# RainbowZL0/swin-unet-image-fusion

Measured on AMD Instinct MI355X. Metric: fused image-pairs/sec at 256x256, win=8, higher is better.
Workload: dtype bf16; 1 GPU; B=16/GPU 256x256 IR/visible pairs, win=8, 5-level Swin-UNet fusion forward (BASELINE configs[1]); global_batch=16, precision_mode=fast, residual_stream=fp32, hip_graph=True, steps_in_flight=3, kernel_schedule=throughput, collective=none, weights=random-init (numpy PCG64 recipe, seed 0)

## Files before the change

include/swinfuse.h:

```cpp
#ifndef SWINFUSE_H
#define SWINFUSE_H

#include <stddef.h>
#include <stdint.h>

#ifdef __cplusplus
extern "C" {
#endif

#define SWF_VERSION_MAJOR 0
#define SWF_VERSION_MINOR 1

typedef void* swf_stream_t;

typedef enum swf_status {
    SWF_OK = 0,
    SWF_ERR_NULL = -1,
    SWF_ERR_BAD_SHAPE = -2,
    SWF_ERR_PAD = -3,
    SWF_ERR_UNSUPPORTED = -4,
    SWF_ERR_WORKSPACE = -5,
    SWF_ERR_HIP = -6
} swf_status;

// ... 207 lines not shown
                const float* x_in, const float* y_in, float* x_out, float* y_out,
                int64_t tokens, int32_t channels, int32_t hidden,
                void* workspace, size_t workspace_bytes, swf_stream_t stream);

int swf_linear_fwd(const swf_linear* lin, const float* in, const float* residual, float* out,
                   int64_t tokens, int32_t n_in, int32_t n_out, int32_t act, swf_stream_t stream);
size_t swf_linear_workspace_bytes(int32_t precision, int64_t tokens, int32_t n_in, int32_t n_out);
int swf_linear_fwd_prec(const swf_linear* lin, int32_t precision, const float* in, const float* residual, float* out,
                        int64_t tokens, int32_t n_in, int32_t n_out, int32_t act,
                        void* workspace, size_t workspace_bytes, swf_stream_t stream);
int swf_layernorm_fwd(const swf_norm* ln, const float* in, float* out, int64_t tokens, int32_t C, int32_t elu,
                      swf_stream_t stream);
int swf_reflect_pad_fwd(const float* in, float* out, int32_t B, int32_t H, int32_t W, int32_t C,
                        int32_t pad_h, int32_t pad_w, swf_stream_t stream);
int swf_crop_fwd(const float* in, float* out, int32_t B, int32_t Hp, int32_t Wp, int32_t H, int32_t W, int32_t C,
                 swf_stream_t stream);

int swf_nchw_to_nhwc(const float* in, float* out, int32_t B, int32_t C, int32_t H, int32_t W, swf_stream_t stream);
int swf_nhwc_to_nchw(const float* in, float* out, int32_t B, int32_t C, int32_t H, int32_t W, swf_stream_t stream);

#define SWF_MAX_LEVELS 8
typedef struct swf_model_desc {
    int32_t levels;
    int32_t in_dims[SWF_MAX_LEVELS];
    int32_t out_dims[SWF_MAX_LEVELS];
    int32_t heads;
    int32_t head_dim[SWF_MAX_LEVELS];
    int32_t mlp_ratio;
    int32_t win_h, win_w, merge_h, merge_w;
    int32_t head_ksize;
    int32_t precision;
    int32_t schedule;
} swf_model_desc;

int32_t swf_model_param_count(const swf_model_desc* desc);
int swf_model_param_info(const swf_model_desc* desc, int32_t index, char* name_buf, size_t name_buf_len,
                         int64_t* offset_elems, int64_t* numel);
int64_t swf_model_arena_elems(const swf_model_desc* desc);
size_t swf_model_workspace_bytes(const swf_model_desc* desc, int32_t B, int32_t H, int32_t W);
int swf_model_forward(const swf_model_desc* desc, const float* arena, const float* ir, const float* vis,
                      float* out, int32_t B, int32_t H, int32_t W,
                      void* workspace, size_t workspace_bytes, swf_stream_t stream);

size_t swf_model_packed_bytes(const swf_model_desc* desc);
int swf_model_pack_weights(const swf_model_desc* desc, const float* arena, void* packed, size_t packed_bytes,
                           swf_stream_t stream);
int swf_model_forward_packed(const swf_model_desc* desc, const float* arena, const void* packed,
                             const float* ir, const float* vis, float* out, int32_t B, int32_t H, int32_t W,
                             void* workspace, size_t workspace_bytes, swf_stream_t stream);

int swf_model_forward_checked(const swf_model_desc* desc, const float* arena, const void* packed,
                              const float* ir, const float* vis, float* out, int32_t B, int32_t H, int32_t W,
                              void* workspace, size_t workspace_bytes, int32_t* cross_equal_flags, swf_stream_t stream);
int swf_model_forward_profiled(const swf_model_desc* desc, const float* arena, const void* packed,
                               const float* ir, const float* vis, float* out, int32_t B, int32_t H, int32_t W,
                               void* workspace, size_t workspace_bytes, float* seg_ms, int32_t seg_count, swf_stream_t stream);
int swf_tensors_equal(const float* a, const float* b, int64_t count, int32_t* flag, swf_stream_t stream);

int swf_bgr8_to_ycrcb_fwd(const uint8_t* bgr, float* y, float* crcb, int32_t B, int32_t H, int32_t W, swf_stream_t stream);
int swf_gray8_to_unit_fwd(const uint8_t* gray, float* out, int64_t count, swf_stream_t stream);
int swf_ycrcb_to_rgb_fwd(const float* fused_y, const float* crcb, float* rgb_f, uint8_t* rgb8,
                         int32_t B, int32_t H, int32_t W, swf_stream_t stream);

typedef struct swf_crop_row {
    uint64_t ir_off;
    uint64_t vis_off;
    int32_t H, W;
    int32_t top, left, h, w;
    int32_t flip;
    int32_t pad_;
} swf_crop_row;
size_t swf_paired_crop_rows_bytes(int32_t B);
int swf_paired_crop_rows_check(const swf_crop_row* rows_host, int32_t B, uint64_t ir_bytes, uint64_t vis_bytes);
int swf_paired_crop_resize_fwd(const uint8_t* ir_base, const uint8_t* vis_base, const swf_crop_row* rows_device, int32_t B,
                               int32_t out_h, int32_t out_w, float* ir_out, float* vis_y_out, swf_stream_t stream);

typedef struct swf_loss_desc {
    int32_t ssim_mode;
    int32_t use_psnr;
    float ir_ssim_weight, ir_psnr_weight;
    float ssim_scale, texture_scale, intensity_scale, psnr_scale;
    float ssim_ratio, texture_ratio, intensity_ratio, psnr_ratio;
} swf_loss_desc;
size_t swf_fusion_loss_workspace_bytes(const swf_loss_desc* desc, int32_t B, int32_t H, int32_t W, int32_t with_grad);
int swf_fusion_loss(const swf_loss_desc* desc, const float* fusion, const float* ir, const float* vis, float* terms, float* grad_fusion,
                    int32_t B, int32_t H, int32_t W, void* workspace, size_t workspace_bytes, swf_stream_t stream);

typedef struct swf_adam_desc {
    double beta1, beta2, eps, weight_decay;
    double max_grad_norm;
    int32_t norm_ready;
} swf_adam_desc;
typedef struct swf_adam_tensor {
    float* param; const float* grad; float* exp_avg; float* exp_avg_sq;
    int64_t numel;
    float step_size;
    float bc2_sqrt;
    int32_t first_chunk;
    int32_t reserved;
} swf_adam_tensor;
size_t swf_adam_table_bytes(int32_t n_tensors, int64_t total_elems);
int swf_adam_table_fill(void* table_host, size_t table_bytes, int32_t n_tensors, const void* const* param, const void* const* grad,
                        const void* const* exp_avg, const void* const* exp_avg_sq, const int64_t* numel, const float* step_size,
                        const float* bc2_sqrt);
int swf_adam_grad_norm(double max_grad_norm, const void* table_pinned_host, void* table_device, size_t table_bytes, int32_t n_tensors,
                       float* norm_out_device, swf_stream_t stream);
// ... 12 lines not shown
```

swin_unet_image_fusion_amd/_lib.py:

```python
from __future__ import annotations

import ctypes as C
import os
from typing import Optional

_HERE = os.path.dirname(os.path.abspath(__file__))
LIB_PATH = os.environ.get("SWF_LIB_PATH") or os.path.join(_HERE, "libswinfuse.so")

SWF_MAX_LEVELS = 8
PREC_FP32, PREC_FAST = 0, 1

OK, ERR_NULL, ERR_BAD_SHAPE, ERR_PAD, ERR_UNSUPPORTED, ERR_WORKSPACE, ERR_HIP = 0, -1, -2, -3, -4, -5, -6

c_float_p = C.c_void_p


class Linear(C.Structure):
    _fields_ = [("weight", C.c_void_p), ("bias", C.c_void_p)]


class Norm(C.Structure):
    _fields_ = [("gamma", C.c_void_p), ("beta", C.c_void_p)]


# ... 102 lines not shown
                                                _vp, _sz, _vp]),
    "swf_window_attention_bwd_drop": (C.c_int, [P(AttnDesc), P(AttnParams), _vp, _vp, _vp, _vp, _vp, _vp, _vp, P(AttnParams), _i32, _i32,
                                                _i32, P(Dropout), _i32, _vp, _sz, _vp]),
    "swf_mlp_drop_workspace_bytes": (_sz, [_i64, _i32, _i32]),
    "swf_mlp_fwd_drop": (C.c_int, [P(Linear), P(Linear), _vp, _vp, _i64, _i32, _i32, P(Dropout), _i32, _vp, _sz, _vp]),
    "swf_mlp_bwd_drop": (C.c_int, [P(Linear), P(Linear), _vp, _vp, _vp, P(Linear), P(Linear), _i64, _i32, _i32, P(Dropout), _i32,
                                   _vp, _sz, _vp]),
    "swf_layernorm_bwd_workspace_bytes": (_sz, [_i64, _i32]),
    "swf_layernorm_bwd": (C.c_int, [P(Norm), _vp, _vp, _vp, P(Norm), _i64, _i32, _vp, _sz, _vp]),
    "swf_patch_layer_bwd_workspace_bytes": (_sz, [_i32] * 8),
    "swf_patch_layer_bwd": (C.c_int, [P(PatchParams), _vp, _vp, _vp, P(PatchParams), _i32, _i32, _i32, _i32, _i32, _i32, _i32, _i32, _vp, _sz, _vp]),
    "swf_reflect_pad_bwd": (C.c_int, [_vp, _vp, _i32, _i32, _i32, _i32, _i32, _i32, _vp]),
    "swf_final_head_bwd_workspace_bytes": (_sz, [_i32, _i32, _i32, _i32]),
    "swf_final_head_bwd": (C.c_int, [P(HeadParams), _vp, _vp, _vp, _vp, _vp, P(HeadGrads), _i32, _i32, _i32, _i32, _i32, _vp, _sz, _vp]),
    "swf_final_head_batch_stats": (C.c_int, [P(HeadParams), _vp, _vp, _vp, _vp, _vp, _vp, C.c_float, _i32, _i32, _i32, _i32, _vp, _sz, _vp]),
    "swf_add_fwd": (C.c_int, [_vp, _vp, _vp, _i64, _vp]),
    "swf_block_pair4_fwd": (C.c_int, [P(BlockDesc), P(BlockStreamParams), P(BlockStreamParams), _vp, _vp, _vp, _vp, _i32, _i32, _i32, _vp, _sz, _vp]),
    "swf_patch_merge_fwd": (C.c_int, [P(PatchParams), _vp, _vp, _i32, _i32, _i32, _i32, _i32, _i32, _i32, _i32, _i32, _vp, _sz, _vp]),
    "swf_merge_out_shape": (C.c_int, [_i32, _i32, _i32, _i32, _i32, _i32, P(_i32), P(_i32), P(_i32), P(_i32)]),
    "swf_patch_unmerge_fwd": (C.c_int, [P(PatchParams), _vp, _vp, _vp, _i32, _i32, _i32, _i32, _i32, _i32, _i32, _i32, _i32, _i32, _i32, _vp, _sz, _vp]),
    "swf_patch_workspace_bytes": (_sz, [_i32] * 10),
    "swf_patch_merge_prec_workspace_bytes": (_sz, [_i32] * 11),
    "swf_patch_merge_fwd_prec": (C.c_int, [_i32, P(PatchParams), P(PatchParams), _vp, _vp, _vp, _vp] + [_i32] * 9
                                 + [P(PatchLn1), P(PatchLn1), P(_i32), _vp, _sz, _vp]),
    "swf_patch_unmerge_prec_workspace_bytes": (_sz, [_i32] * 13),
    "swf_patch_unmerge_fwd_prec": (C.c_int, [_i32, P(PatchParams), P(PatchParams), _vp, _vp, _vp, _vp, _vp, _vp] + [_i32] * 11
                                   + [P(PatchLn1), P(PatchLn1), P(_i32), _vp, _sz, _vp]),
    "swf_final_head_fwd": (C.c_int, [P(HeadParams), _vp, _vp, _vp, _i32, _i32, _i32, _i32, _vp, _sz, _vp]),
    "swf_linear_fwd": (C.c_int, [P(Linear), _vp, _vp, _vp, _i64, _i32, _i32, _i32, _vp]),
    "swf_mlp_workspace_bytes": (_sz, [_i32, _i64, _i32, _i32]),
    "swf_mlp_fwd": (C.c_int, [_i32, P(BlockStreamParams), P(BlockStreamParams), _vp, _vp, _vp, _vp, _i64, _i32, _i32, _vp, _sz, _vp]),
    "swf_linear_workspace_bytes": (_sz, [_i32, _i64, _i32, _i32]),
    "swf_linear_fwd_prec": (C.c_int, [P(Linear), _i32, _vp, _vp, _vp, _i64, _i32, _i32, _i32, _vp, _sz, _vp]),
    "swf_layernorm_fwd": (C.c_int, [P(Norm), _vp, _vp, _i64, _i32, _i32, _vp]),
    "swf_reflect_pad_fwd": (C.c_int, [_vp, _vp, _i32, _i32, _i32, _i32, _i32, _i32, _vp]),
    "swf_crop_fwd": (C.c_int, [_vp, _vp, _i32, _i32, _i32, _i32, _i32, _i32, _vp]),
    "swf_nchw_to_nhwc": (C.c_int, [_vp, _vp, _i32, _i32, _i32, _i32, _vp]),
    "swf_nhwc_to_nchw": (C.c_int, [_vp, _vp, _i32, _i32, _i32, _i32, _vp]),
    "swf_bgr8_to_ycrcb_fwd": (C.c_int, [_vp, _vp, _vp, _i32, _i32, _i32, _vp]),
    "swf_gray8_to_unit_fwd": (C.c_int, [_vp, _vp, _i64, _vp]),
    "swf_ycrcb_to_rgb_fwd": (C.c_int, [_vp, _vp, _vp, _vp, _i32, _i32, _i32, _vp]),
    "swf_paired_crop_rows_bytes": (_sz, [_i32]),
    "swf_paired_crop_rows_check": (C.c_int, [_vp, _i32, C.c_uint64, C.c_uint64]),
    "swf_paired_crop_resize_fwd": (C.c_int, [_vp, _vp, _vp, _i32, _i32, _i32, _vp, _vp, _vp]),
    "swf_model_param_count": (_i32, [P(ModelDesc)]),
    "swf_model_param_info": (C.c_int, [P(ModelDesc), _i32, C.c_char_p, _sz, P(_i64), P(_i64)]),
    "swf_model_arena_elems": (_i64, [P(ModelDesc)]),
    "swf_model_workspace_bytes": (_sz, [P(ModelDesc), _i32, _i32, _i32]),
    "swf_model_forward": (C.c_int, [P(ModelDesc), _vp, _vp, _vp, _vp, _i32, _i32, _i32, _vp, _sz, _vp]),
    "swf_model_packed_bytes": (_sz, [P(ModelDesc)]),
    "swf_model_pack_weights": (C.c_int, [P(ModelDesc), _vp, _vp, _sz, _vp]),
    "swf_model_forward_packed": (C.c_int, [P(ModelDesc), _vp, _vp, _vp, _vp, _vp, _i32, _i32, _i32, _vp, _sz, _vp]),
    "swf_model_forward_checked": (C.c_int, [P(ModelDesc), _vp, _vp, _vp, _vp, _vp, _i32, _i32, _i32, _vp, _sz, _vp, _vp]),
    "swf_model_forward_profiled": (C.c_int, [P(ModelDesc), _vp, _vp, _vp, _vp, _vp, _i32, _i32, _i32, _vp, _sz, P(C.c_float), _i32, _vp]),
    "swf_tensors_equal": (C.c_int, [_vp, _vp, _i64, _vp, _vp]),
    "swf_fusion_loss_workspace_bytes": (_sz, [P(LossDesc), _i32, _i32, _i32, _i32]),
    "swf_fusion_loss": (C.c_int, [P(LossDesc), _vp, _vp, _vp, _vp, _vp, _i32, _i32, _i32, _vp, _sz, _vp]),
    "swf_adam_table_bytes": (_sz, [_i32, _i64]),
    "swf_adam_table_fill": (C.c_int, [_vp, _sz, _i32, _vp, _vp, _vp, _vp, _vp, _vp, _vp]),
    "swf_adam_grad_norm": (C.c_int, [C.c_double, _vp, _vp, _sz, _i32, _vp, _vp]),
    "swf_adam_step": (C.c_int, [P(AdamDesc), _vp, _vp, _sz, _i32, _vp, _vp]),
}

_lib: Optional[C.CDLL] = None


class SwinFuseLibraryMissing(ImportError):
    pass


def lib() -> C.CDLL:
    global _lib
    if _lib is None:
        if not os.path.exists(LIB_PATH):
            raise SwinFuseLibraryMissing(
                f"{LIB_PATH} not found: build the HIP extension first "
                "(python -c 'import __graft_entry__ as g; g.build()').  There is no CPU fallback.")
        handle = C.CDLL(LIB_PATH)
        for name, (res, args) in SIGNATURES.items():
            fn = getattr(handle, name)
            fn.restype = res
            fn.argtypes = args
        _lib = handle
    return _lib


def check(status: int) -> None:
    if status == OK:
        return
    msg = lib().swf_last_error_string().decode(errors="replace")
    kind = lib().swf_status_string(status).decode()
    text = f"libswinfuse: {kind}: {msg}"
    if status == ERR_BAD_SHAPE:
        raise ValueError(text)
    if status == ERR_UNSUPPORTED:
        raise NotImplementedError(text)
    raise RuntimeError(text)
```

swin_unet_image_fusion_amd/csrc/kernels_patchrr.h:

```cpp
#pragma once
#include "kernels_patch.h"

namespace swf {

bool patch_rr_supported(int decoder, int Cin, int Cout, int mh, int mw);
size_t patch_rr_packed_bytes(int decoder, int Cin, int Cout, int mh, int mw);
int pack_patch_rr(int decoder, int Cin, int Cout, int mh, int mw, const float* weight, const float* bias, const float* gamma,
                  const float* beta, void* dst, hipStream_t stream);
int launch_patch_rr(const PatchFusedDesc& d, const void* const* packed, int nstream, hipStream_t stream);

}
```

swin_unet_image_fusion_amd/csrc/kernels_patchrr.hip:

```cpp
#include "kernels_patchrr.h"

#include <algorithm>

#include "win_frag.h"

namespace swf {
namespace {

using namespace wf;

struct PrrArgs {
    const float* in[2]; float* out[2]; const float* skip[2]; const char* packed[2];
    int B, H, W, Cin;
    int mh, mw, Hm, Wm;
    int Ho, Wo;
    int K, N, Cout, M;
};

template <int KS, int NT>
struct PRR {
    static constexpr int NFRAG = NT * KS * 2;
    static constexpr int NV = NT * 16;
    static constexpr size_t p_vec = size_t(NFRAG) * 1024;
    static constexpr size_t p_total = p_vec + size_t(3) * 2 * NV * 4;
// ... 158 lines not shown
            for (int nt = 0; nt < NT; ++nt)
#pragma unroll
                for (int i = 0; i < 16; ++i) {
                    const float d = acc[u][nt][i] - mean;
                    q += (32 * nt + rho(i, hf) < N) ? d * d : 0.f;
                }
            const float rstd = __builtin_amdgcn_rsqf(sum_halves(q) * invN + 1e-5f);
            const int t = tok[u];
            if constexpr (DEC_VEC) {
                if (a.Cout > 1) {
                    if constexpr (!SKIP_EARLY) load_skips(u);
                }
            }
#pragma unroll
            for (int nt = 0; nt < NT; ++nt)
#pragma unroll
                for (int g = 0; g < 4; ++g) {
                    const int n0 = 32 * nt + 8 * g + 4 * hf;
                    if (n0 < N) {
                        float y[4];
#pragma unroll
                        for (int j = 0; j < 4; ++j) {
                            const int i = 4 * g + j;
                            const float z = (acc[u][nt][i] - mean) * rstd * vgam[nt * 16 + i] + vbet[nt * 16 + i];
                            y[j] = z > 0.f ? z : __builtin_amdgcn_exp2f(z * kLog2e) - 1.0f;
                        }
                        if constexpr (!DEC) {
                            if (live[u]) *reinterpret_cast<float4*>(a.out[s] + (int64_t)t * N + n0) = make_float4(y[0], y[1], y[2], y[3]);
                        } else if (a.Cout == 1) {
                            if (live[u]) {
                                const int mx = t % a.Wm, t2 = t / a.Wm, my = t2 % a.Hm, b = t2 / a.Hm;
#pragma unroll
                                for (int j = 0; j < 4; ++j) {
                                    const int yy = my * 2 + (j >> 1), xx = mx * 2 + (j & 1);
                                    if (yy < a.Ho && xx < a.Wo) {
                                        const int64_t o = ((int64_t)b * a.Ho + yy) * a.Wo + xx;
                                        a.out[s][o] = a.skip[s] ? y[j] + a.skip[s][o] : y[j];
                                    }
                                }
                            }
                        } else {
                            const int o = oidx[u][nt][g];
                            if (o >= 0) {
                                const float4 k4 = skv[u][nt][g];
                                *reinterpret_cast<float4*>(a.out[s] + o) = make_float4(y[0] + k4.x, y[1] + k4.y, y[2] + k4.z, y[3] + k4.w);
                            }
                        }
                    }
                }
        }
    }
}

struct PrrPackArgs { const float* w; const float* bias; const float* gamma; const float* beta; char* dst; int K, N; };

template <int KS, int NT>
__global__ __launch_bounds__(256) void patch_rr_pack_kernel(PrrPackArgs a) {
    using P = PRR<KS, NT>;
    const int gtid = blockIdx.x * blockDim.x + threadIdx.x, gsz = gridDim.x * blockDim.x;
    for (int idx = gtid; idx < P::NFRAG * 512; idx += gsz) {
        const int f = idx >> 9, lane = (idx >> 3) & 63, e = idx & 7, r = lane & 31, hf = lane >> 5;
        const int hl = f & 1, ks = (f >> 1) % KS, nt = f / (2 * KS);
        const int n = 32 * nt + r, k = 16 * ks + 8 * hf + e;
        const float val = (n < a.N && k < a.K) ? a.w[(int64_t)n * a.K + k] : 0.f;
        const bf16 hi = (bf16)val;
        reinterpret_cast<bf16*>(a.dst)[idx] = hl ? (bf16)(val - (float)hi) : hi;
    }
    float* vec = reinterpret_cast<float*>(a.dst + P::p_vec);
    for (int i = gtid; i < 3 * 2 * P::NV; i += gsz) {
        const int which = i / (2 * P::NV), hf = (i / P::NV) & 1, j = i % P::NV, nt = j >> 4, reg = j & 15;
        const int n = 32 * nt + rho(reg, hf);
        const float* src = which == 0 ? a.bias : which == 1 ? a.gamma : a.beta;
        vec[i] = (n < a.N && src) ? src[n] : 0.f;
    }
}

bool shape_class(int decoder, int Cin, int Cout, int mh, int mw, int* ks, int* nt) {
    if (mh != 2 || mw != 2 || Cin <= 0 || Cout <= 0) return false;
    const int K = decoder ? Cin : 4 * Cin, N = decoder ? 4 * Cout : Cout;
    if (decoder) {
        if (Cin % 8 || !(Cout == 1 || Cout % 4 == 0)) return false;
    } else {
        if (!(Cin == 1 || Cin % 8 == 0) || Cout % 4) return false;
    }
    *ks = (K + 15) / 16;
    *nt = (N + 31) / 32;
    const int k = *ks, n = *nt;
    if (decoder) return (k == 2 && n == 1) || (k == 3 && n == 3) || (k == 6 && n == 6);
    return (k == 1 && n == 1 && Cin == 1) || (k == 6 && n == 2) || (k == 12 && n == 3);
}

template <int KS, int NT, int DEC, int CIN1, int TPW>
int launch_t(const PrrArgs& a, int nstream, hipStream_t stream) {
    const int ngroup = (a.M + 32 * TPW - 1) / (32 * TPW);
    const int gx = std::max(1, std::min((ngroup + 3) / 4, 8 * num_cus() / nstream));
    hipLaunchKernelGGL((patch_rr_kernel<KS, NT, DEC, CIN1, TPW>), dim3(gx, nstream), dim3(256), 0, stream, a);
    return check_launch("patch_rr");
}

}

bool patch_rr_supported(int decoder, int Cin, int Cout, int mh, int mw) {
    int ks, nt;
    return shape_class(decoder, Cin, Cout, mh, mw, &ks, &nt);
}

size_t patch_rr_packed_bytes(int decoder, int Cin, int Cout, int mh, int mw) {
    int ks, nt;
    if (!shape_class(decoder, Cin, Cout, mh, mw, &ks, &nt)) return 0;
    return align_up(size_t(nt) * ks * 2 * 1024 + size_t(3) * 2 * nt * 16 * 4, 256);
}

int pack_patch_rr(int decoder, int Cin, int Cout, int mh, int mw, const float* weight, const float* bias, const float* gamma,
                  const float* beta, void* dst, hipStream_t stream) {
    int ks, nt;
    if (!shape_class(decoder, Cin, Cout, mh, mw, &ks, &nt)) return fail(SWF_ERR_UNSUPPORTED, "pack_patch_rr: shape not covered");
    PrrPackArgs a{weight, bias, gamma, beta, static_cast<char*>(dst), decoder ? Cin : 4 * Cin, decoder ? 4 * Cout : Cout};
#define SWF_PRR_PACK(KS_, NT_) if (ks == KS_ && nt == NT_) { hipLaunchKernelGGL((patch_rr_pack_kernel<KS_, NT_>), dim3(32), dim3(256), 0, stream, a); return check_launch("pack_patch_rr"); }
    SWF_PRR_PACK(1, 1) SWF_PRR_PACK(2, 1) SWF_PRR_PACK(3, 3) SWF_PRR_PACK(6, 2) SWF_PRR_PACK(6, 6) SWF_PRR_PACK(12, 3)
#undef SWF_PRR_PACK
    return fail(SWF_ERR_UNSUPPORTED, "pack_patch_rr: shape class");
}

int launch_patch_rr(const PatchFusedDesc& d, const void* const* packed, int nstream, hipStream_t stream) {
    int ks, nt;
    if (!shape_class(d.decoder, d.Cin, d.Cout, d.mh, d.mw, &ks, &nt)) return fail(SWF_ERR_UNSUPPORTED, "patch_rr: shape not covered");
    if (d.M <= 0 || d.M > INT32_MAX - 64) return fail(SWF_ERR_UNSUPPORTED, "patch_rr: token count");
    const int64_t in_elems = (int64_t)d.B * d.H * d.W * d.Cin;
    const int64_t out_elems = d.decoder ? (int64_t)d.B * d.Ho * d.Wo * d.Cout : d.M * (int64_t)d.N;
    if (in_elems >= (int64_t(1) << 31) || out_elems >= (int64_t(1) << 31)) return fail(SWF_ERR_UNSUPPORTED, "patch_rr: tensor too large");
    PrrArgs a{};
    uintptr_t bits = 0;
    for (int s = 0; s < nstream; ++s) {
        if (!packed || !packed[s]) return fail(SWF_ERR_NULL, "patch_rr: packed image missing");
        a.in[s] = d.in[s]; a.out[s] = d.out[s]; a.skip[s] = d.skip[s]; a.packed[s] = static_cast<const char*>(packed[s]);
        bits |= reinterpret_cast<uintptr_t>(d.in[s]) | reinterpret_cast<uintptr_t>(d.out[s]) | reinterpret_cast<uintptr_t>(d.skip[s]) |
                reinterpret_cast<uintptr_t>(packed[s]);
    }
    if (bits % 16) return fail(SWF_ERR_UNSUPPORTED, "patch_rr: tensors must be 16-byte aligned");
    a.B = d.B; a.H = d.H; a.W = d.W; a.Cin = d.Cin; a.mh = d.mh; a.mw = d.mw; a.Hm = d.Hm; a.Wm = d.Wm; a.Ho = d.Ho; a.Wo = d.Wo;
    a.K = d.K; a.N = d.N; a.Cout = d.Cout; a.M = (int)d.M;
    if (!d.decoder) {
        if (ks == 1 && nt == 1 && d.Cin == 1) return launch_t<1, 1, 0, 1, 2>(a, nstream, stream);
        if (ks == 6 && nt == 2) return launch_t<6, 2, 0, 0, 2>(a, nstream, stream);
        if (ks == 12 && nt == 3) return launch_t<12, 3, 0, 0, 1>(a, nstream, stream);
    } else {
        if (ks == 2 && nt == 1) return launch_t<2, 1, 1, 0, 2>(a, nstream, stream);
        if (ks == 3 && nt == 3) return launch_t<3, 3, 1, 0, 1>(a, nstream, stream);
        if (ks == 6 && nt == 6) return launch_t<6, 6, 1, 0, 1>(a, nstream, stream);
    }
    return fail(SWF_ERR_UNSUPPORTED, "patch_rr: no instantiation for k-steps %d, tiles %d (decoder %d)", ks, nt, d.decoder);
}

}
```

swin_unet_image_fusion_amd/csrc/kernels_win24.hip:

```cpp
#include "win_host.h"

namespace swf {
namespace {

using namespace wf;

constexpr int W24_WAVES = 3;

template <int HID_>
struct G24 {
    static constexpr int C = 24, HID = HID_, HEADS = 8, D = 3;
    static constexpr bool ONES_H = HID % 32 != 0;
    static constexpr int NT1 = (HID + (ONES_H ? 1 : 0) + 31) / 32;
    static constexpr int KU = (HID + (ONES_H ? 1 : 0) + 15) / 16;
    static constexpr int F_QKV = 0;
    static constexpr int F_P = 12;
    static constexpr int F_W1 = 16;
    static constexpr int F_W2 = F_W1 + 4 * NT1;
    static constexpr int NFRAG = F_W2 + 2 * KU;
    static constexpr size_t p_vec = size_t(NFRAG) * 1024;
    static constexpr int V_LN1G = 0, V_LN1B = 12, V_LN2G = 24, V_LN2B = 36, V_B2 = 48;
    static constexpr size_t p_bias = p_vec + 2 * 64 * 4;
    static constexpr size_t p_total = p_bias + size_t(2) * 2 * 16 * 64 * 4;
    static constexpr size_t l_k = 0, l_v = l_k + 16 * 1024, l_vec = l_v + 16 * 1024, l_total = l_vec + 2 * 2 * 64 * 4;
    static constexpr size_t p_total16 = p_bias + size_t(15) * 64 * 16 * 4;
    static constexpr size_t l_k16 = 0, l_v16 = 32 * 1024, l_vec16 = 64 * 1024, l_total16 = l_vec16 + 2 * 2 * 64 * 4;
};

__device__ __forceinline__ void layernorm_frags(const f32x16& res, const float* vec, int goff, int boff, u32x4 (&xh)[2], u32x4 (&xl)[2]) {
    float s = 0.f;
#pragma unroll
    for (int i = 0; i < 12; ++i) s += res[i];
    const float mean = sum_halves(s) * (1.0f / 24.0f);
    float d[12], q = 0.f;
#pragma unroll
    for (int i = 0; i < 12; ++i) {
        d[i] = res[i] - mean;
        q += d[i] * d[i];
    }
    const float rstd = __builtin_amdgcn_rsqf(sum_halves(q) * (1.0f / 24.0f) + 1e-5f);
    float n[16];
#pragma unroll
    for (int a = 0; a < 3; ++a) {
        const float4 g = *reinterpret_cast<const float4*>(vec + goff + 4 * a);
        const float4 b = *reinterpret_cast<const float4*>(vec + boff + 4 * a);
        n[4 * a + 0] = d[4 * a + 0] * rstd * g.x + b.x;
        n[4 * a + 1] = d[4 * a + 1] * rstd * g.y + b.y;
        n[4 * a + 2] = d[4 * a + 2] * rstd * g.z + b.z;
        n[4 * a + 3] = d[4 * a + 3] * rstd * g.w + b.w;
    }
    n[12] = 1.0f;
    n[13] = n[14] = n[15] = 0.f;
    split8(n, xh[0], xl[0]);
    split8(n + 8, xh[1], xl[1]);
}

__device__ __forceinline__ void raw_frags(const f32x16& res, u32x4 (&xh)[2], u32x4 (&xl)[2]) {
    float n[16];
#pragma unroll
    for (int i = 0; i < 12; ++i) n[i] = res[i];
// ... 43 lines not shown
            float p[8];
#pragma unroll
            for (int j = 0; j < 8; ++j) p[j] = __builtin_amdgcn_exp2f((ps >> 1) ? s1[8 * (ps & 1) + j] : s0[8 * (ps & 1) + j]);
            const u32x4 pf = pack8_f16(p);
            const u32x4 va = vsrc[ps * 64];
            t = mfma_f16(va, pf, ps == 0 ? zero16 : t);
            __builtin_amdgcn_sched_barrier(0);
        }
#pragma unroll
        for (int j = 0; j < 4; ++j) {
            const int i = 4 * (h >> 1) + j;
            o[i] = keep ? (ONLINE ? __builtin_fmaf(o[i], alpha, t[i]) : t[i]) : o[i];
        }
        __builtin_amdgcn_sched_barrier(0);
    }
    return o;
}

__device__ __forceinline__ void load_rows24(const __amdgpu_buffer_rsrc_t& irs, unsigned tokoff, f32x16& dstv) {
#pragma unroll
    for (int a = 0; a < 3; ++a) {
        const f32x4 v = __builtin_bit_cast(f32x4, __builtin_amdgcn_raw_buffer_load_b128(irs, tokoff, 32 * a, 0));
        dstv[4 * a] = v.x; dstv[4 * a + 1] = v.y; dstv[4 * a + 2] = v.z; dstv[4 * a + 3] = v.w;
    }
    dstv[12] = dstv[13] = dstv[14] = dstv[15] = 0.f;
}
__device__ __forceinline__ void store_rows24(__amdgpu_buffer_rsrc_t ors, unsigned tokoff, f32x16 res) {
#pragma unroll
    for (int a = 0; a < 3; ++a) {
        const f32x4 v = {res[4 * a], res[4 * a + 1], res[4 * a + 2], res[4 * a + 3]};
        __builtin_amdgcn_raw_buffer_store_b128(__builtin_bit_cast(u32x4, v), ors, tokoff, 32 * a, 0);
    }
}

template <class G, class WFn>
__device__ __forceinline__ f32x16 project24(WFn WF, f32x16 o, f32x16 res) {
    float t[16];
#pragma unroll
    for (int a = 0; a < 4; ++a) {
        const float inv = __builtin_amdgcn_rcpf(o[4 * a + 3]);
        t[4 * a] = o[4 * a] * inv; t[4 * a + 1] = o[4 * a + 1] * inv; t[4 * a + 2] = o[4 * a + 2] * inv;
        t[4 * a + 3] = 1.0f;
    }
    u32x4 oh[2], ol[2];
    split8(t, oh[0], ol[0]);
    split8(t + 8, oh[1], ol[1]);
    SWF_WF_FENCE();
#pragma unroll
    for (int s = 0; s < 2; ++s) res = mma3(WF(G::F_P + 2 * s), WF(G::F_P + 2 * s + 1), oh[s], ol[s], res);
    return res;
}


template <int HID, int WS, int MODE = WIN_BLOCK, bool RAW = false>
__global__ __launch_bounds__(256, W24_WAVES) void window24_kernel(WinArgs args) {
    using G = G24<HID>;
    static_assert(WS == 7 || WS == 8, "window side");
    static_assert(MODE == WIN_BLOCK || MODE == WIN_ATTN || MODE == WIN_MLP, "mode");
    static_assert(!RAW || MODE != WIN_BLOCK, "RAW belongs to the half-block modes");
    constexpr bool ATT = MODE != WIN_MLP, MLP = MODE != WIN_ATTN;
    __shared__ __attribute__((aligned(16))) char smem[G::l_total];
    u32x4* kimg = reinterpret_cast<u32x4*>(smem + G::l_k);
    u32x4* vimg = reinterpret_cast<u32x4*>(smem + G::l_v);
    float* lvec = reinterpret_cast<float*>(smem + G::l_vec);

    const int tid = threadIdx.x, lane = tid & 63, wave = tid >> 6;
    const int ws = wave >> 1, qb = wave & 1, r = lane & 31, hf = lane >> 5;
    const int H = args.H, W = args.W, nwx = MLP && !ATT ? 1 : W / WS, nwy = MLP && !ATT ? 1 : H / WS, npi = nwx * nwy;
    const int nwin = ATT ? args.B * npi : (max(args.ntok[0], args.ntok[1]) + 63) / 64;
    const int sh = args.shift ? WS / 2 : 0;
    const int kvs = args.cross ? 1 - ws : ws;

    for (int i = tid; i < 2 * 2 * 64; i += 256) lvec[i] = reinterpret_cast<const float*>(args.packed[i >> 7] + G::p_vec)[i & 127];
    const __amdgpu_buffer_rsrc_t wrs = __builtin_amdgcn_make_buffer_rsrc(const_cast<char*>(uniform_ptr(args.packed[ws])), 0, (int)G::p_total, 0x00020000);
    const __amdgpu_buffer_rsrc_t krs = __builtin_amdgcn_make_buffer_rsrc(const_cast<char*>(uniform_ptr(args.packed[kvs])), 0, (int)G::p_total, 0x00020000);
    const int act_bytes = ATT ? args.B * H * W * 24 * 4 : args.ntok[ws] * 24 * 4;
    const __amdgpu_buffer_rsrc_t irs = __builtin_amdgcn_make_buffer_rsrc(const_cast<float*>(uniform_ptr(args.in[ws])), 0, act_bytes, 0x00020000);
    const __amdgpu_buffer_rsrc_t ors = __builtin_amdgcn_make_buffer_rsrc(uniform_ptr(args.out[ws]), 0, (MODE == WIN_BLOCK || args.out[ws]) ? act_bytes : 0, 0x00020000);
    const unsigned loff = (unsigned)lane * 16u;
    auto WF = [&](int f) { return __builtin_bit_cast(u32x4, __builtin_amdgcn_raw_buffer_load_b128(wrs, loff, f * 1024, 0)); };
    auto WK = [&](int f) { return __builtin_bit_cast(u32x4, __builtin_amdgcn_raw_buffer_load_b128(krs, loff, f * 1024, 0)); };
    const float* vec = lvec + (ws * 2 + hf) * 64;
    f32x16 bias[2];
    auto load_bias = [&]() {
        const int vo = lane * 128 + qb * (2 * 16 * 64 * 4);
#pragma unroll
        for (int kt = 0; kt < 2; ++kt)
#pragma unroll
            for (int q4 = 0; q4 < 4; ++q4) {
                const f32x4 t = __builtin_bit_cast(f32x4, __builtin_amdgcn_raw_buffer_load_b128(wrs, vo + (kt * 16 + q4 * 4) * 4, (int)G::p_bias, 0));
#pragma unroll
                for (int e = 0; e < 4; ++e) bias[kt][q4 * 4 + e] = t[e];
            }
    };
    if constexpr (ATT) load_bias();
    const bool half1 = hf != 0;
    const bool col_masked = half1 != (((r >> 2) & 1) != 0);
    __syncthreads();

    int it = 0;
    for (int win = blockIdx.x; win < nwin; win += gridDim.x, ++it) {
        SWF_WF_FENCE();
        const int b = win / npi, wrem = win - b * npi;
        const int wy = wrem / nwx, wx = wrem - wy * nwx;
        const int buf = it & 1;
        int lane_w = lane;
        asm volatile("" : "+v"(lane_w));
        const int ty = 4 * qb + ((lane_w >> 3) & 3), tx = lane_w & 7;
        unsigned oy = wy * WS + ty + sh, ox = wx * WS + tx + sh;
        oy = oy < oy - (unsigned)H ? oy : oy - (unsigned)H;
        ox = ox < ox - (unsigned)W ? ox : ox - (unsigned)W;
        const unsigned tokoff = [&]() -> unsigned {
            if constexpr (ATT) {
                return (WS == 8 || (ty < WS && tx < WS)) ? (unsigned)((((b * H + (int)oy) * W + (int)ox) * 24 + 4 * (lane_w >> 5)) * 4) : 0x80000000u;
            } else {
                const int tok = 64 * win + 32 * qb + (lane_w & 31);
                return tok < args.ntok[ws] ? (unsigned)((tok * 24 + 4 * (lane_w >> 5)) * 4) : 0x80000000u;
            }
        }();
        const f32x16 zero16 = {0.f, 0.f, 0.f, 0.f, 0.f, 0.f, 0.f, 0.f, 0.f, 0.f, 0.f, 0.f, 0.f, 0.f, 0.f, 0.f};

        f32x16 res;
        if constexpr (ATT) {
        u32x4 qf[2];
        {
            f32x16 x0;
            load_rows24(irs, tokoff, x0);
            u32x4 xh[2], xl[2];
            if constexpr (RAW) raw_frags(x0, xh, xl);
            else layernorm_frags(x0, vec, G::V_LN1G, G::V_LN1B, xh, xl);
            f32x16 acc = zero16;
            if (!(RAW && ws == 1)) {
#pragma unroll
                for (int s = 0; s < 2; ++s) acc = mma3(WF(G::F_QKV + 2 * s), WF(G::F_QKV + 2 * s + 1), xh[s], xl[s], acc);
                float t[16];
#pragma unroll
                for (int i = 0; i < 16; ++i) t[i] = acc[i];
                qf[0] = pack8_f16(t);
                qf[1] = pack8_f16(t + 8);
            }
            SWF_WF_FENCE();
            if (!(RAW && ws == 0)) {
                float t[16];
                acc = zero16;
#pragma unroll
                for (int s = 0; s < 2; ++s) acc = mma3(WK(G::F_QKV + 4 + 2 * s), WK(G::F_QKV + 5 + 2 * s), xh[s], xl[s], acc);
#pragma unroll
                for (int i = 0; i < 16; ++i) t[i] = acc[i];
                u32x4* kdst = kimg + (((buf * 2 + kvs) * 2 + qb) * 2) * 64 + lane;
                kdst[0] = pack8_f16(t);
// ... 19 lines not shown
            const u32x4* vsrc = vimg + ((buf * 2 + ws) * 4) * 64 + lane;
            if (rowv || colv) {
                const float pen0 = ((rowv && qb == 1) || (colv && col_masked)) ? -INFINITY : 0.f;
                const float pen1 = ((rowv && qb == 0) || (colv && col_masked)) ? -INFINITY : 0.f;
#pragma unroll
                for (int i = 0; i < 16; ++i) { bias[0][i] += pen0; bias[1][i] += pen1; }
            }
            o = attention24<false>(ksrc, vsrc, qf, bias, half1, zero16);
            if (rowv || colv) load_bias();
        }

        SWF_WF_FENCE();
        if constexpr (RAW) res = zero16;
        else load_rows24(irs, tokoff, res);
        res = project24<G>(WF, o, res);
        } else {
            load_rows24(irs, tokoff, res);
        }

        if constexpr (MLP) {
            u32x4 xh[2], xl[2];
            if constexpr (RAW) { raw_frags(res, xh, xl); res = zero16; }
            else layernorm_frags(res, vec, G::V_LN2G, G::V_LN2B, xh, xl);
#pragma unroll
            for (int tI = 0; tI < G::NT1; ++tI) {
                SWF_WF_FENCE();
                f32x16 acc = zero16;
#pragma unroll
                for (int s = 0; s < 2; ++s)
                    acc = mma3(WF(G::F_W1 + 4 * tI + 2 * s), WF(G::F_W1 + 4 * tI + 2 * s + 1), xh[s], xl[s], acc);
                float e[16];
                elu_tile(acc, e);
#pragma unroll
                for (int s2 = 0; s2 < 2; ++s2) {
                    const int u = 2 * tI + s2;
                    if (u < G::KU) {
                        u32x4 hh, hl;
                        split8(e + 8 * s2, hh, hl);
                        SWF_WF_FENCE();
                        res = mma3(WF(G::F_W2 + 2 * u), WF(G::F_W2 + 2 * u + 1), hh, hl, res);
                    }
                }
                __builtin_amdgcn_sched_barrier(0);
            }
            if constexpr (!G::ONES_H) {
#pragma unroll
                for (int a = 0; a < 3; ++a) {
                    const float4 b2 = *reinterpret_cast<const float4*>(vec + G::V_B2 + 4 * a);
                    res[4 * a] += b2.x; res[4 * a + 1] += b2.y; res[4 * a + 2] += b2.z; res[4 * a + 3] += b2.w;
                }
            }
        }

        store_rows24(ors, tokoff, res);
    }

    if (args.warm[0]) warm_next_block<256>(args, tid);
}

template <int HID>
__global__ __launch_bounds__(256, 2) void window24w16_kernel(WinArgs args) {
    using G = G24<HID>;
    extern __shared__ __attribute__((aligned(16))) char smem16[];
    u32x4* kimg = reinterpret_cast<u32x4*>(smem16 + G::l_k16);
    u32x4* vimg = reinterpret_cast<u32x4*>(smem16 + G::l_v16);
    float* lvec = reinterpret_cast<float*>(smem16 + G::l_vec16);

    const int tid = threadIdx.x, lane = tid & 63, wave = tid >> 6;
    const int ws = wave >> 1, pw = wave & 1, r = lane & 31, hf = lane >> 5;
    const int H = args.H, W = args.W, nwx = W / 16, nwy = H / 16, npi = nwx * nwy;
    const int nwin = args.B * npi;
    const int sh = args.shift ? 8 : 0;
    const int kvs = args.cross ? 1 - ws : ws;

    for (int i = tid; i < 2 * 2 * 64; i += 256) lvec[i] = reinterpret_cast<const float*>(args.packed[i >> 7] + G::p_vec)[i & 127];
    const __amdgpu_buffer_rsrc_t wrs = __builtin_amdgcn_make_buffer_rsrc(const_cast<char*>(uniform_ptr(args.packed[ws])), 0, (int)G::p_total16, 0x00020000);
    const __amdgpu_buffer_rsrc_t krs = __builtin_amdgcn_make_buffer_rsrc(const_cast<char*>(uniform_ptr(args.packed[kvs])), 0, (int)G::p_total16, 0x00020000);
    const int act_bytes = args.B * H * W * 24 * 4;
    const __amdgpu_buffer_rsrc_t irs = __builtin_amdgcn_make_buffer_rsrc(const_cast<float*>(uniform_ptr(args.in[ws])), 0, act_bytes, 0x00020000);
    const __amdgpu_buffer_rsrc_t ors = __builtin_amdgcn_make_buffer_rsrc(uniform_ptr(args.out[ws]), 0, act_bytes, 0x00020000);
    const unsigned loff = (unsigned)lane * 16u;
    auto WF = [&](int f) { return __builtin_bit_cast(u32x4, __builtin_amdgcn_raw_buffer_load_b128(wrs, loff, f * 1024, 0)); };
    auto WK = [&](int f) { return __builtin_bit_cast(u32x4, __builtin_amdgcn_raw_buffer_load_b128(krs, loff, f * 1024, 0)); };
    const float* vec = lvec + (ws * 2 + hf) * 64;
    const bool half1 = hf != 0;
    const f32x16 zero16 = {0.f, 0.f, 0.f, 0.f, 0.f, 0.f, 0.f, 0.f, 0.f, 0.f, 0.f, 0.f, 0.f, 0.f, 0.f, 0.f};
    __syncthreads();

    for (int win = blockIdx.x; win < nwin; win += gridDim.x) {
        SWF_WF_FENCE();
        const int b = win / npi, wrem = win - b * npi;
        const int wy = wrem / nwx, wx = wrem - wy * nwx;
        auto tokoff_of = [&](int j) {
            int lane_w = lane;
            asm volatile("" : "+v"(lane_w));
            unsigned oy = wy * 16 + 2 * j + ((lane_w >> 4) & 1) + sh, ox = wx * 16 + (lane_w & 15) + sh;
            oy = oy < oy - (unsigned)H ? oy : oy - (unsigned)H;
            ox = ox < ox - (unsigned)W ? ox : ox - (unsigned)W;
            return (unsigned)((((b * H + (int)oy) * W + (int)ox) * 24 + 4 * (lane_w >> 5)) * 4);
        };

        u32x4 qf[4][2];
#pragma unroll
        for (int q = 0; q < 4; ++q) { qf[q][0] = u32x4{0u, 0u, 0u, 0u}; qf[q][1] = u32x4{0u, 0u, 0u, 0u}; }
        {
            u32x4 wq[4], wk[4], wv[4];
#pragma unroll
// ... 123 lines not shown
        if (f < G::F_P) {
            const int t = f >> 2, st = (f >> 1) & 1;
            hl = f & 1;
            const int k = rho(8 * st + e, hf), head = r >> 2, c = r & 3;
            const swf_linear& l = t == 0 ? p.attn.q : t == 1 ? p.attn.k : p.attn.v;
            if (c < 3) {
                const int row = 3 * head + c;
                val = k < 24 ? lin(l, row, k, 24) : (k == 24 ? pack_bia(l, row) : 0.f);
                if (t == 0) val *= qscale;
            } else if (t != 0 && k == 24) {
                val = 1.0f;
            }
        } else if (f < G::F_W1) {
            const int st = ((f - G::F_P) >> 1) & 1;
            hl = f & 1;
            const int k = rho(8 * st + e, hf), head = k >> 2, c = k & 3;
            if (r < 24) val = c < 3 ? lin(p.attn.proj, r, 3 * head + c, 24) : (k == 3 ? pack_bia(p.attn.proj, r) : 0.f);
        } else if (f < G::F_W2) {
            const int g = f - G::F_W1, t = g >> 2, st = (g >> 1) & 1;
            hl = g & 1;
            const int k = rho(8 * st + e, hf), hid = 32 * t + r;
            if (hid < HID) val = (k < 24 ? lin(p.fc1, hid, k, 24) : (k == 24 ? pack_bia(p.fc1, hid) : 0.f)) * kLog2e;
            else if (G::ONES_H && hid == HID && k == 24) val = 1.0f;
        } else {
            const int g = f - G::F_W2, u = g >> 1;
            hl = g & 1;
            const int hid = 32 * (u >> 1) + rho(8 * (u & 1) + e, hf);
            if (r < 24) val = hid < HID ? lin(p.fc2, r, hid, HID) * kLn2 : ((G::ONES_H && hid == HID) ? pack_bia(p.fc2, r) : 0.f);
        }
        const bf16 hi = (bf16)val;
        reinterpret_cast<bf16*>(dst)[idx] = hl ? (bf16)(val - (float)hi) : hi;
    }
    float* vec = reinterpret_cast<float*>(dst + G::p_vec);
    for (int i = gtid; i < 128; i += gsz) {
        const int hf = i >> 6, j = i & 63, which = j / 12, k = j % 12;
        const int c = 8 * (k >> 2) + 4 * hf + (k & 3);
        float v = 0.f;
        if (which == 0) v = p.ln1.gamma ? p.ln1.gamma[c] : 1.f;
        else if (which == 1) v = p.ln1.beta ? p.ln1.beta[c] : 0.f;
        else if (which == 2) v = p.ln2.gamma ? p.ln2.gamma[c] : 1.f;
        else if (which == 3) v = p.ln2.beta ? p.ln2.beta[c] : 0.f;
        else if (which == 4) v = (p.fc2.weight && p.fc2.bias) ? p.fc2.bias[c] : 0.f;
        vec[i] = v;
    }
    if (p.attn.bias_table) pack_rel_bias<true>(reinterpret_cast<float*>(dst + G::p_bias), p.attn.bias_table, a.ws, gtid, gsz);
}

struct L24 {
    static constexpr int C = 24, D = 3, HID_WIDE = 96, HID_NARROW = 4, PACK_GRID = 32, WAVES = W24_WAVES;
    static constexpr const char *name = "win24", *pack_name = "pack_win24";
    template <int HID> using G = G24<HID>;
    template <int HID>
    static void pack(dim3 grid, const WinPackArgs& a, hipStream_t stream) { hipLaunchKernelGGL((pack24_kernel<HID>), grid, dim3(256), 0, stream, a); }
    template <int HID, int WS, int MODE, bool RAW>
    static int launch(const swf_block_desc&, const WinArgs& a, int grid, hipStream_t stream) {
        hipLaunchKernelGGL((window24_kernel<HID, WS, MODE, RAW>), dim3(grid), dim3(256), 0, stream, a);
        return check_launch(MODE == WIN_BLOCK ? "window24" : "window24 (half block)");
    }
    template <int HID>
    static int launch16(const WinArgs& a, int nwin, hipStream_t stream) {
        constexpr int lds = (int)G24<HID>::l_total16;
        SWF_TRY(raise_lds_limit<&window24w16_kernel<HID>>(lds, "window24w16"));
        hipLaunchKernelGGL((window24w16_kernel<HID>), dim3(std::min(nwin, 2 * num_cus())), dim3(256), lds, stream, a);
        return check_launch("window24w16");
    }
};

}

const WinLevel& win24_level() {
    static const WinLevel level = win_level<L24>();
    return level;
}

}
```

swin_unet_image_fusion_amd/csrc/kernels_win48.hip:

```cpp
#include "win_host.h"

namespace swf {
namespace {

using namespace wf;

constexpr int W48_WAVES = 2;

template <int HID_>
struct G48 {
    static constexpr int C = 48, HID = HID_, HEADS = 8, D = 6;
    static constexpr int NT1 = HID / 32, KU = HID / 16;
    static_assert(HID % 32 == 0, "hidden tiles");
    static constexpr int F_QKV = 0;
    static constexpr int F_P = 36;
    static constexpr int F_W1 = 52;
    static constexpr int F_W2 = F_W1 + 6 * NT1;
    static constexpr int NFRAG = F_W2 + 4 * KU;
    static constexpr int V_LN1G = 0, V_LN1B = 24, V_LN2G = 48, V_LN2B = 72, V_B2 = 96, V_BQ = 120, V_BK = 152, V_B1 = 184, VHF = 288;
    static_assert(V_B1 + 16 * NT1 <= VHF, "vector block");
    static constexpr int VSTREAM = 2 * VHF + 64;
    static constexpr size_t p_vec = size_t(NFRAG) * 1024;
    static constexpr size_t p_bias = (p_vec + size_t(VSTREAM) * 4 + 15) / 16 * 16;
    static constexpr size_t p_total = p_bias + size_t(2) * 2 * 16 * 64 * 4;
    static constexpr size_t l_k = 0, l_v = 16 * 1024, l_vec = 32 * 1024, l_total = l_vec + size_t(2) * VSTREAM * 4;
    static constexpr size_t p_total16 = p_bias + size_t(15) * 16 * 64 * 4;
    static constexpr size_t l_k16 = 0, l_v16 = 32 * 1024, l_vec16 = 64 * 1024, l_total16 = l_vec16 + size_t(2) * VSTREAM * 4;
};


__device__ __forceinline__ void raw48(const f32x16& x0, const f32x16& x1, u32x4 (&xh)[3], u32x4 (&xl)[3]) {
    float n[24];
#pragma unroll
    for (int i = 0; i < 24; ++i) n[i] = i < 16 ? x0[i] : x1[i - 16];
    split8(n, xh[0], xl[0]);
    split8(n + 8, xh[1], xl[1]);
    split8(n + 16, xh[2], xl[2]);
}

__device__ __forceinline__ void layernorm48(const f32x16& x0, const f32x16& x1, const float* vec, int goff, int boff, u32x4 (&xh)[3], u32x4 (&xl)[3]) {
    float s = 0.f;
#pragma unroll
    for (int i = 0; i < 16; ++i) s += x0[i];
#pragma unroll
    for (int i = 0; i < 8; ++i) s += x1[i];
    const float mean = sum_halves(s) * (1.0f / 48.0f);
    float d[24], q = 0.f;
#pragma unroll
    for (int i = 0; i < 24; ++i) {
        d[i] = (i < 16 ? x0[i] : x1[i - 16]) - mean;
        q += d[i] * d[i];
    }
    const float rstd = __builtin_amdgcn_rsqf(sum_halves(q) * (1.0f / 48.0f) + 1e-5f);
    float n[24];
#pragma unroll
    for (int a = 0; a < 6; ++a) {
        const float4 g = *reinterpret_cast<const float4*>(vec + goff + 4 * a);
        const float4 b = *reinterpret_cast<const float4*>(vec + boff + 4 * a);
        n[4 * a + 0] = d[4 * a + 0] * rstd * g.x + b.x;
        n[4 * a + 1] = d[4 * a + 1] * rstd * g.y + b.y;
// ... 12 lines not shown
    if constexpr (!ONLINE) { o[0] = zero16; o[1] = zero16; }
#pragma unroll
    for (int h = 0; h < 8; ++h) {
        const int T = h >> 2, hq = h & 3, sp = hq >> 1, sub = hq & 1;
        const u32x4 ka0 = ksrc[((0 * 2 + T) * 2 + sp) * 64], ka1 = ksrc[((1 * 2 + T) * 2 + sp) * 64];
        u32x4 qm = {0u, 0u, 0u, 0u};
        qm[2 * sub] = qf[T][sp][2 * sub];
        qm[2 * sub + 1] = qf[T][sp][2 * sub + 1];
        float mx;
        {
            f32x16 s0 = mfma_f16(ka0, qm, bias[0]);
            mx = max3f(s0[0], s0[1], s0[2]);
#pragma unroll
            for (int i = 3; i < 15; i += 2) mx = max3f(mx, s0[i], s0[i + 1]);
            mx = __builtin_fmaxf(mx, s0[15]);
        }
        {
            f32x16 s1 = mfma_f16(ka1, qm, bias[1]);
#pragma unroll
            for (int i = 0; i < 16; i += 2) mx = max3f(mx, s1[i], s1[i + 1]);
        }
        mx = max_halves(mx);
        f16 nm = (f16)(-mx);
        float alpha = 0.f;
        if constexpr (ONLINE) {
            const float mold = mrun[h];
            nm = (f16)(-__builtin_fmaxf(mold, mx));
            const float mnew = -(float)nm;
            alpha = __builtin_amdgcn_exp2f(mold - mnew);
            mrun[h] = mnew;
        }
        qm[2 * sub + 1] |= half1 ? ((unsigned)__builtin_bit_cast(unsigned short, nm) << 16) : 0u;
        f32x16 t;
#pragma unroll
        for (int kt = 0; kt < 2; ++kt) {
            f32x16 sc = mfma_f16(kt ? ka1 : ka0, qm, bias[kt]);
#pragma unroll
            for (int s2 = 0; s2 < 2; ++s2) {
                float p[8];
#pragma unroll
                for (int j = 0; j < 8; ++j) p[j] = __builtin_amdgcn_exp2f(sc[8 * s2 + j]);
                const u32x4 pf = pack8_f16(p);
                const u32x4 va = vsrc[(T * VSTEPS + 2 * kt + s2) * 64];
                t = mfma_f16(va, pf, (kt == 0 && s2 == 0) ? zero16 : t);
                __builtin_amdgcn_sched_barrier(0);
            }
        }
#pragma unroll
        for (int j = 0; j < 4; ++j) o[T][4 * hq + j] = ONLINE ? __builtin_fmaf(o[T][4 * hq + j], alpha, t[4 * hq + j]) : t[4 * hq + j];
        __builtin_amdgcn_sched_barrier(0);
    }
}

template <int HID, int WS, int MODE = WIN_BLOCK, bool RAW = false>
__global__ __launch_bounds__(256, W48_WAVES) void window48_kernel(WinArgs args) {
    using G = G48<HID>;
    static_assert(WS == 7 || WS == 8, "window side");
    static_assert(!RAW || MODE != WIN_BLOCK, "RAW belongs to the half-block modes");
    constexpr bool ATT = MODE != WIN_MLP, MLP = MODE != WIN_ATTN;
    __shared__ __attribute__((aligned(16))) char smem[G::l_total];
    u32x4* kimg = reinterpret_cast<u32x4*>(smem + G::l_k);
    u32x4* vimg = reinterpret_cast<u32x4*>(smem + G::l_v);
    float* lvec = reinterpret_cast<float*>(smem + G::l_vec);

    const int tid = threadIdx.x, lane = tid & 63, wave = tid >> 6;
    const int ws = wave >> 1, qb = wave & 1, r = lane & 31, hf = lane >> 5;
    const int H = args.H, W = args.W, nwx = ATT ? W / WS : 1, nwy = ATT ? H / WS : 1, npi = nwx * nwy;
    const int nwin = ATT ? args.B * npi : (max(args.ntok[0], args.ntok[1]) + 63) / 64;
    const int sh = args.shift ? WS / 2 : 0;
    const int kvs = args.cross ? 1 - ws : ws;

    const __amdgpu_buffer_rsrc_t wrs = __builtin_amdgcn_make_buffer_rsrc(const_cast<char*>(uniform_ptr(args.packed[ws])), 0, (int)G::p_total, 0x00020000);
    const __amdgpu_buffer_rsrc_t krs = __builtin_amdgcn_make_buffer_rsrc(const_cast<char*>(uniform_ptr(args.packed[kvs])), 0, (int)G::p_total, 0x00020000);
    const int act_bytes = ATT ? args.B * H * W * 48 * 4 : args.ntok[ws] * 48 * 4;
    const __amdgpu_buffer_rsrc_t irs = __builtin_amdgcn_make_buffer_rsrc(const_cast<float*>(uniform_ptr(args.in[ws])), 0, act_bytes, 0x00020000);
    const __amdgpu_buffer_rsrc_t ors = __builtin_amdgcn_make_buffer_rsrc(uniform_ptr(args.out[ws]), 0, (MODE == WIN_BLOCK || args.out[ws]) ? act_bytes : 0, 0x00020000);
    const unsigned loff = (unsigned)lane * 16u;
    auto WF = [&](int f) { return __builtin_bit_cast(u32x4, __builtin_amdgcn_raw_buffer_load_b128(wrs, loff, f * 1024, 0)); };
    auto WK = [&](int f) { return __builtin_bit_cast(u32x4, __builtin_amdgcn_raw_buffer_load_b128(krs, loff, f * 1024, 0)); };
    const float* vec = lvec + ws * G::VSTREAM + hf * G::VHF;
    const float* veck = lvec + kvs * G::VSTREAM + hf * G::VHF;
    const float* vecv = lvec + kvs * G::VSTREAM + 2 * G::VHF;
    const bool half1 = hf != 0;
    const bool col_masked = half1 != (((r >> 2) & 1) != 0);
    const f32x16 zero16 = {0.f, 0.f, 0.f, 0.f, 0.f, 0.f, 0.f, 0.f, 0.f, 0.f, 0.f, 0.f, 0.f, 0.f, 0.f, 0.f};

    for (int win = blockIdx.x; win < nwin; win += gridDim.x) {
        SWF_WF_FENCE();
        const int b = win / npi, wrem = win - b * npi;
        const int wy = wrem / nwx, wx = wrem - wy * nwx;
        const int ty = 4 * qb + (r >> 3), tx = r & 7;
        int oy = wy * WS + ty + sh, ox = wx * WS + tx + sh;
        oy = oy >= H ? oy - H : oy;
        ox = ox >= W ? ox - W : ox;
        const unsigned tokoff = [&]() -> unsigned {
            if constexpr (ATT) {
                return (WS == 8 || (ty < WS && tx < WS)) ? (unsigned)((((b * H + oy) * W + ox) * 48 + 4 * hf) * 4) : 0x80000000u;
            } else {
                const int tok = 64 * win + 32 * qb + r;
                return tok < args.ntok[ws] ? (unsigned)((tok * 48 + 4 * hf) * 4) : 0x80000000u;
            }
        }();
        auto load_rows = [&](f32x16& t0, f32x16& t1) {
#pragma unroll
            for (int a = 0; a < 6; ++a) {
                const f32x4 v = __builtin_bit_cast(f32x4, __builtin_amdgcn_raw_buffer_load_b128(irs, tokoff, 32 * a, 0));
                if (a < 4) { t0[4 * a] = v.x; t0[4 * a + 1] = v.y; t0[4 * a + 2] = v.z; t0[4 * a + 3] = v.w; }
                else { t1[4 * (a - 4)] = v.x; t1[4 * (a - 4) + 1] = v.y; t1[4 * (a - 4) + 2] = v.z; t1[4 * (a - 4) + 3] = v.w; }
            }
#pragma unroll
            for (int i = 8; i < 16; ++i) t1[i] = 0.f;
        };

        f32x16 res0, res1;
        if constexpr (ATT) {
        u32x4 qf[2][2];
        {
            u32x4 wq[2][6];
            auto req = [&](int ph, u32x4 (&dst)[6]) {
                const int m = ph >> 1, T = ph & 1;
#pragma unroll
                for (int i = 0; i < 6; ++i) dst[i] = m == 0 ? WF(G::F_QKV + ((m * 2 + T) * 3) * 2 + i) : WK(G::F_QKV + ((m * 2 + T) * 3) * 2 + i);
            };
            req(0, wq[0]);
            f32x16 x0, x1;
            load_rows(x0, x1);
            if (win == (int)blockIdx.x) {
                static_assert(G::VSTREAM % 4 == 0 && G::p_vec % 16 == 0, "vector sections move as 16-byte groups");
                    fill_vectors<G::VSTREAM / 4, 256>(lvec, args.packed[0] + G::p_vec, args.packed[1] + G::p_vec, tid);
                __syncthreads();
            }
            u32x4 xh[3], xl[3];
            if constexpr (RAW) raw48(x0, x1, xh, xl);
            else layernorm48(x0, x1, vec, G::V_LN1G, G::V_LN1B, xh, xl);
            float t[16];
#pragma unroll
            for (int ph = 0; ph < 6; ++ph) {
                const int m = ph >> 1, T = ph & 1;
                SWF_WF_FENCE();
                if (ph + 1 < 6) req(ph + 1, wq[(ph + 1) & 1]);
                SWF_WF_FENCE();
                const u32x4 (&w)[6] = wq[ph & 1];
                f32x16 acc = zero16;
                if (RAW && (m == 0 ? ws == 1 : ws == 0)) {
                    if (ph == 2 && win != (int)blockIdx.x) __syncthreads();
                } else if (m < 2) {
#pragma unroll
                    for (int s = 0; s < 3; ++s) acc = mma3(w[2 * s], w[2 * s + 1], xh[s], xl[s], acc);
                    const float* bsrc = m == 0 ? vec + G::V_BQ : veck + G::V_BK;
#pragma unroll
                    for (int g = 0; g < 4; ++g) {
                        const float4 bb = *reinterpret_cast<const float4*>(bsrc + 16 * T + 4 * g);
                        t[4 * g] = acc[4 * g] + bb.x; t[4 * g + 1] = acc[4 * g + 1] + bb.y; t[4 * g + 2] = acc[4 * g + 2] + bb.z; t[4 * g + 3] = acc[4 * g + 3] + bb.w;
                    }
                    if (m == 0) {
                        qf[T][0] = pack8_f16(t);
                        qf[T][1] = pack8_f16(t + 8);
                    } else {
                        if (T == 0 && win != (int)blockIdx.x) __syncthreads();
                        u32x4* kdst = kimg + (((kvs * 2 + qb) * 2 + T) * 2) * 64 + lane;
                        kdst[0] = pack8_f16(t);
                        kdst[64] = pack8_f16(t + 8);
                    }
                } else {
#pragma unroll
                    for (int s = 0; s < 3; ++s) acc = mma3(xh[s], xl[s], w[2 * s], w[2 * s + 1], acc);
                    const float bv = vecv[32 * T + r];
#pragma unroll
                    for (int i = 0; i < 16; ++i) t[i] = acc[i] + bv;
                    u32x4* vdst = vimg + ((kvs * 2 + T) * 4 + 2 * qb) * 64 + lane;
                    vdst[0] = pack8_f16(t);
                    vdst[64] = pack8_f16(t + 8);
                }
            }
        }
        f32x16 bias[2];
        load_bias_tiles(wrs, loff, (int)G::p_bias, __builtin_amdgcn_readfirstlane(qb) * 2, bias);
        __syncthreads();
        if (RAW && ws == 1) continue;

        f32x16 o[2];
        {
            const bool rowv = args.shift && wy == nwy - 1, colv = args.shift && wx == nwx - 1;
            const u32x4* ksrc = kimg + (ws * 8) * 64 + lane;
            const u32x4* vsrc = vimg + (ws * 8) * 64 + lane;
            if (rowv || colv) {
                const float pen0 = ((rowv && qb == 1) || (colv && col_masked)) ? -INFINITY : 0.f;
                const float pen1 = ((rowv && qb == 0) || (colv && col_masked)) ? -INFINITY : 0.f;
#pragma unroll
                for (int i = 0; i < 16; ++i) { bias[0][i] += pen0; bias[1][i] += pen1; }
            }
            attention48<false>(ksrc, vsrc, qf, bias, half1, o);
        }

        u32x4 wpj[16];
        SWF_WF_FENCE();
        if constexpr (RAW) { res0 = zero16; res1 = zero16; }
        else load_rows(res0, res1);
#pragma unroll
        for (int i = 0; i < 16; ++i) wpj[i] = WF(G::F_P + i);
        SWF_WF_FENCE();
        {
            u32x4 oh[4], ol[4];
#pragma unroll
            for (int T = 0; T < 2; ++T) {
                float t[16];
#pragma unroll
                for (int q = 0; q < 4; ++q) {
                    float lo_, den;
                    halves(o[T][4 * q + 2], lo_, den);
                    const float inv = __builtin_amdgcn_rcpf(den);
                    t[4 * q] = o[T][4 * q] * inv; t[4 * q + 1] = o[T][4 * q + 1] * inv; t[4 * q + 2] = o[T][4 * q + 2] * inv; t[4 * q + 3] = o[T][4 * q + 3] * inv;
                }
                split8(t, oh[2 * T], ol[2 * T]);
                split8(t + 8, oh[2 * T + 1], ol[2 * T + 1]);
            }
#pragma unroll
            for (int ks = 0; ks < 4; ++ks) {
                res0 = mma3(wpj[(0 * 4 + ks) * 2], wpj[(0 * 4 + ks) * 2 + 1], oh[ks], ol[ks], res0);
                res1 = mma3(wpj[(1 * 4 + ks) * 2], wpj[(1 * 4 + ks) * 2 + 1], oh[ks], ol[ks], res1);
            }
        }

        } else {
            load_rows(res0, res1);
            if (win == (int)blockIdx.x) {
                fill_vectors<G::VSTREAM / 4, 256>(lvec, args.packed[0] + G::p_vec, args.packed[1] + G::p_vec, tid);
                __syncthreads();
            }
        }

        if constexpr (MLP) {
            u32x4 w1[2][6];
            auto req1 = [&](int tI, u32x4 (&dst)[6]) {
#pragma unroll
                for (int i = 0; i < 6; ++i) dst[i] = WF(G::F_W1 + tI * 6 + i);
            };
            u32x4 w2[2][2][2][2];
            auto req2 = [&](int tI, u32x4 (&dst)[2][2][2]) {
#pragma unroll
                for (int To = 0; To < 2; ++To)
#pragma unroll
                    for (int s2 = 0; s2 < 2; ++s2) {
                        dst[To][s2][0] = WF(G::F_W2 + (To * G::KU + 2 * tI + s2) * 2);
                        dst[To][s2][1] = WF(G::F_W2 + (To * G::KU + 2 * tI + s2) * 2 + 1);
                    }
            };
            req1(0, w1[0]);
            req2(0, w2[0]);
            u32x4 xh[3], xl[3];
            if constexpr (RAW) { raw48(res0, res1, xh, xl); res0 = zero16; res1 = zero16; }
            else layernorm48(res0, res1, vec, G::V_LN2G, G::V_LN2B, xh, xl);
#pragma unroll
            for (int tI = 0; tI < G::NT1; ++tI) {
                SWF_WF_FENCE();
                if (tI + 1 < G::NT1) { req1(tI + 1, w1[(tI + 1) & 1]); req2(tI + 1, w2[(tI + 1) & 1]); }
                SWF_WF_FENCE();
                const u32x4 (&w)[6] = w1[tI & 1];
                f32x16 acc = zero16;
#pragma unroll
                for (int s = 0; s < 3; ++s) acc = mma3(w[2 * s], w[2 * s + 1], xh[s], xl[s], acc);
                float e[16];
                elu_tile(acc, vec + G::V_B1 + 16 * tI, e);
#pragma unroll
                for (int s2 = 0; s2 < 2; ++s2) {
                    u32x4 hh, hl;
                    split8(e + 8 * s2, hh, hl);
                    res0 = mma3(w2[tI & 1][0][s2][0], w2[tI & 1][0][s2][1], hh, hl, res0);
                    res1 = mma3(w2[tI & 1][1][s2][0], w2[tI & 1][1][s2][1], hh, hl, res1);
                }
                __builtin_amdgcn_sched_barrier(0);
            }
#pragma unroll
            for (int a = 0; a < 6; ++a) {
                const float4 b2 = *reinterpret_cast<const float4*>(vec + G::V_B2 + 4 * a);
                if (a < 4) { res0[4 * a] += b2.x; res0[4 * a + 1] += b2.y; res0[4 * a + 2] += b2.z; res0[4 * a + 3] += b2.w; }
                else { res1[4 * (a - 4)] += b2.x; res1[4 * (a - 4) + 1] += b2.y; res1[4 * (a - 4) + 2] += b2.z; res1[4 * (a - 4) + 3] += b2.w; }
            }
        }

#pragma unroll
        for (int a = 0; a < 6; ++a) {
            const f32x4 v = a < 4 ? f32x4{res0[4 * a], res0[4 * a + 1], res0[4 * a + 2], res0[4 * a + 3]}
                                  : f32x4{res1[4 * (a - 4)], res1[4 * (a - 4) + 1], res1[4 * (a - 4) + 2], res1[4 * (a - 4) + 3]};
            __builtin_amdgcn_raw_buffer_store_b128(__builtin_bit_cast(u32x4, v), ors, tokoff, 32 * a, 0);
        }
    }

    if (args.warm[0]) warm_next_block<256>(args, tid);
}

template <int HID>
__global__ __launch_bounds__(256, 2) void window48w16_kernel(WinArgs args) {
    using G = G48<HID>;
    extern __shared__ __attribute__((aligned(16))) char smem48[];
    u32x4* kimg = reinterpret_cast<u32x4*>(smem48 + G::l_k16);
    u32x4* vimg = reinterpret_cast<u32x4*>(smem48 + G::l_v16);
    float* lvec = reinterpret_cast<float*>(smem48 + G::l_vec16);

    const int tid = threadIdx.x, lane = tid & 63, wave = tid >> 6;
    const int ws = blockIdx.y, r = lane & 31, hf = lane >> 5;
    const int H = args.H, W = args.W, nwx = W / 16, nwy = H / 16, npi = nwx * nwy;
    const int nwin = args.B * npi;
    const int sh = args.shift ? 8 : 0;
    const int src = args.cross ? 1 - ws : ws;

    static_assert(G::VSTREAM % 4 == 0 && G::p_vec % 16 == 0, "vector sections move as 16-byte groups");
                    fill_vectors<G::VSTREAM / 4, 256>(lvec, args.packed[0] + G::p_vec, args.packed[1] + G::p_vec, tid);
    const __amdgpu_buffer_rsrc_t wrs = __builtin_amdgcn_make_buffer_rsrc(const_cast<char*>(args.packed[ws]), 0, (int)G::p_total16, 0x00020000);
    const int act_bytes = args.B * H * W * 48 * 4;
    const __amdgpu_buffer_rsrc_t irs = __builtin_amdgcn_make_buffer_rsrc(const_cast<float*>(args.in[ws]), 0, act_bytes, 0x00020000);
    const __amdgpu_buffer_rsrc_t srs = __builtin_amdgcn_make_buffer_rsrc(const_cast<float*>(args.in[src]), 0, act_bytes, 0x00020000);
    const __amdgpu_buffer_rsrc_t ors = __builtin_amdgcn_make_buffer_rsrc(args.out[ws], 0, act_bytes, 0x00020000);
    const unsigned loff = (unsigned)lane * 16u;
    auto WF = [&](int f) { return __builtin_bit_cast(u32x4, __builtin_amdgcn_raw_buffer_load_b128(wrs, loff, f * 1024, 0)); };
    const float* vec = lvec + ws * G::VSTREAM + hf * G::VHF;
    const float* vecs = lvec + src * G::VSTREAM + hf * G::VHF;
    const float* vecv = lvec + ws * G::VSTREAM + 2 * G::VHF;
    const bool half1 = hf != 0;
    const f32x16 zero16 = {0.f, 0.f, 0.f, 0.f, 0.f, 0.f, 0.f, 0.f, 0.f, 0.f, 0.f, 0.f, 0.f, 0.f, 0.f, 0.f};
    __syncthreads();

    for (int win = blockIdx.x; win < nwin; win += gridDim.x) {
        SWF_WF_FENCE();
        const int b = win / npi, wrem = win - b * npi;
        const int wy = wrem / nwx, wx = wrem - wy * nwx;
        auto tokoff_of = [&](int j) {
            int oy = wy * 16 + 2 * j + (r >> 4) + sh, ox = wx * 16 + (r & 15) + sh;
            oy = oy >= H ? oy - H : oy;
            ox = ox >= W ? ox - W : ox;
            return (unsigned)((((b * H + oy) * W + ox) * 48 + 4 * hf) * 4);
        };
        auto load_rows = [&](const __amdgpu_buffer_rsrc_t& rs, unsigned tokoff, f32x16& t0, f32x16& t1) {
#pragma unroll
            for (int a = 0; a < 6; ++a) {
                const f32x4 v = __builtin_bit_cast(f32x4, __builtin_amdgcn_raw_buffer_load_b128(rs, tokoff, 32 * a, 0));
                if (a < 4) { t0[4 * a] = v.x; t0[4 * a + 1] = v.y; t0[4 * a + 2] = v.z; t0[4 * a + 3] = v.w; }
                else { t1[4 * (a - 4)] = v.x; t1[4 * (a - 4) + 1] = v.y; t1[4 * (a - 4) + 2] = v.z; t1[4 * (a - 4) + 3] = v.w; }
// ... 198 lines not shown
        } else if (f < G::F_W1) {
            const int g = (f - G::F_P) >> 1, ks = g & 3, To = g >> 2;
            hl = f & 1;
            const int n = 32 * To + r, v = kslot(ks, hf, e), head = v >> 3, c = v & 7;
            if (n < 48) val = c < 6 ? pack_wgt(p.attn.proj, n * 48 + head * 6 + c) : (v == 6 ? pack_bia(p.attn.proj, n) : 0.f);
        } else if (f < G::F_W2) {
            const int g = (f - G::F_W1) >> 1, s = g % 3, tI = g / 3;
            hl = f & 1;
            const int k = kslot(s, hf, e), hid = 32 * tI + r;
            if (k < 48) val = pack_wgt(p.fc1, hid * 48 + k) * kLog2e;
        } else {
            const int g = (f - G::F_W2) >> 1, u = g % G::KU, To = g / G::KU;
            hl = f & 1;
            const int n = 32 * To + r, hid = kslot(u, hf, e);
            if (n < 48) val = pack_wgt(p.fc2, n * HID + hid) * kLn2;
        }
        const bf16 hi = (bf16)val;
        reinterpret_cast<bf16*>(dst)[idx] = hl ? (bf16)(val - (float)hi) : hi;
    }
    float* vec = reinterpret_cast<float*>(dst + G::p_vec);
    for (int i = gtid; i < G::VSTREAM; i += gsz) {
        float v = 0.f;
        if (i < 2 * G::VHF) {
            const int hf = i / G::VHF, j = i % G::VHF;
            if (j < G::V_BQ) {
                const int which = j / 24, k = j % 24;
                const int c = k < 16 ? rho(k, hf) : 32 + rho(k - 16, hf);
                v = which == 0 ? (p.ln1.gamma ? p.ln1.gamma[c] : 1.f) : which == 1 ? (p.ln1.beta ? p.ln1.beta[c] : 0.f)
                  : which == 2 ? (p.ln2.gamma ? p.ln2.gamma[c] : 1.f) : which == 3 ? (p.ln2.beta ? p.ln2.beta[c] : 0.f) : pack_bia(p.fc2, c);
            } else if (j < G::V_B1) {
                const int isk = j >= G::V_BK, k = (j - (isk ? G::V_BK : G::V_BQ)), T = k >> 4, vch = 32 * T + rho(k & 15, hf);
                const int head = vch >> 3, c = vch & 7;
                if (c < 6) v = isk ? pack_bia(p.attn.k, head * 6 + c) : pack_bia(p.attn.q, head * 6 + c) * qscale;
                else if (isk && c == 7) v = 1.0f;
            } else if (j < G::V_B1 + 16 * G::NT1) {
                const int k = j - G::V_B1, hid = 32 * (k >> 4) + rho(k & 15, hf);
                v = pack_bia(p.fc1, hid) * kLog2e;
            }
        } else {
            const int vch = i - 2 * G::VHF, head = vch >> 3, c = vch & 7;
            v = c < 6 ? pack_bia(p.attn.v, head * 6 + c) : (c == 6 ? 1.0f : 0.f);
        }
        vec[i] = v;
    }
    if (p.attn.bias_table) pack_rel_bias<false>(reinterpret_cast<float*>(dst + G::p_bias), p.attn.bias_table, a.ws, gtid, gsz);
}

struct L48 {
    static constexpr int C = 48, D = 6, HID_WIDE = 192, HID_NARROW = 96, PACK_GRID = 64, WAVES = W48_WAVES;
    static constexpr const char *name = "win48", *pack_name = "pack_win48";
    template <int HID> using G = G48<HID>;
    template <int HID>
    static void pack(dim3 grid, const WinPackArgs& a, hipStream_t stream) { hipLaunchKernelGGL((pack48_kernel<HID>), grid, dim3(256), 0, stream, a); }
    template <int HID, int WS, int MODE, bool RAW>
    static int launch(const swf_block_desc&, const WinArgs& a, int grid, hipStream_t stream) {
        hipLaunchKernelGGL((window48_kernel<HID, WS, MODE, RAW>), dim3(grid), dim3(256), 0, stream, a);
        return check_launch(MODE == WIN_BLOCK ? "window48" : "window48 (half block)");
    }
    template <int HID>
    static int launch16(const WinArgs& a, int nwin, hipStream_t stream) {
        constexpr int lds = (int)G48<HID>::l_total16;
        SWF_TRY(raise_lds_limit<&window48w16_kernel<HID>>(lds, "window48w16"));
        hipLaunchKernelGGL((window48w16_kernel<HID>), dim3(std::min(nwin, num_cus()), 2), dim3(256), lds, stream, a);
        return check_launch("window48w16");
    }
};

}

const WinLevel& win48_level() {
    static const WinLevel level = win_level<L48>();
    return level;
}

}
```

swin_unet_image_fusion_amd/csrc/kernels_win96.hip:

```cpp
#include "win_host.h"

#include <cstdlib>

namespace swf {
namespace {

using namespace wf;

template <int HID_>
struct G96 {
    static constexpr int C = 96, HID = HID_, HEADS = 8, D = 12, TC = 3, VT = 4, KS = 6;
    static constexpr int NT1 = HID / 32, KU = HID / 16;
    static_assert(HID % 32 == 0, "hidden tiles");
    static constexpr int F_QKV = 0;
    static constexpr int F_P = 144;
    static constexpr int F_W1 = 192;
    static constexpr int F_W2 = F_W1 + 12 * NT1;
    static constexpr int NFRAG = F_W2 + 6 * KU;
    static constexpr int V_LN1G = 0, V_LN1B = 48, V_LN2G = 96, V_LN2B = 144, V_B2 = 192, V_BQ = 240, V_BK = 304, V_B1 = 368;
    static constexpr int VHF = V_B1 + 16 * NT1, VSTREAM = 2 * VHF + 128;
    static constexpr size_t p_vec = size_t(NFRAG) * 1024;
    static constexpr size_t p_bias = (p_vec + size_t(VSTREAM) * 4 + 15) / 16 * 16;
    static constexpr size_t p_total = p_bias + size_t(2) * 2 * 16 * 64 * 4;
    static constexpr size_t l_k = 0, l_v = 32 * 1024, l_vec = 64 * 1024, l_total = l_vec + size_t(2) * VSTREAM * 4;
// ... 935 lines not shown
                val = pack_wgt(l, (head * 12 + c) * 96 + k);
                if (m == 0) val *= qscale;
            }
        } else if (f < G::F_W1) {
            const int g = (f - G::F_P) >> 1, ks = g & 7, To = g >> 3;
            const int n = 32 * To + r, row = rho(e, hf);
            val = row < 12 ? pack_wgt(p.attn.proj, n * 96 + ks * 12 + row) : ((ks == 0 && row == 12) ? pack_bia(p.attn.proj, n) : 0.f);
        } else if (f < G::F_W2) {
            const int g = (f - G::F_W1) >> 1, s = g % 6, tI = g / 6;
            const int k = kslot(s, hf, e), hid = 32 * tI + r;
            val = pack_wgt(p.fc1, hid * 96 + k) * kLog2e;
        } else {
            const int g = (f - G::F_W2) >> 1, u = g % G::KU, To = g / G::KU;
            const int n = 32 * To + r, hid = kslot(u, hf, e);
            val = pack_wgt(p.fc2, n * HID + hid) * kLn2;
        }
        const bf16 hi = (bf16)val;
        reinterpret_cast<bf16*>(dst)[idx] = hl ? (bf16)(val - (float)hi) : hi;
    }
    float* vec = reinterpret_cast<float*>(dst + G::p_vec);
    for (int i = gtid; i < G::VSTREAM; i += gsz) {
        float v = 0.f;
        if (i < 2 * G::VHF) {
            const int hf = i / G::VHF, j = i % G::VHF;
            if (j < G::V_BQ) {
                const int which = j / 48, k = j % 48;
                const int c = 32 * (k >> 4) + rho(k & 15, hf);
                v = which == 0 ? (p.ln1.gamma ? p.ln1.gamma[c] : 1.f) : which == 1 ? (p.ln1.beta ? p.ln1.beta[c] : 0.f)
                  : which == 2 ? (p.ln2.gamma ? p.ln2.gamma[c] : 1.f) : which == 3 ? (p.ln2.beta ? p.ln2.beta[c] : 0.f) : pack_bia(p.fc2, c);
            } else if (j < G::V_B1) {
                const int isk = j >= G::V_BK, k = j - (isk ? G::V_BK : G::V_BQ), vch = 32 * (k >> 4) + rho(k & 15, hf);
                const int head = vch >> 4, c = vch & 15;
                if (c < 12) v = isk ? pack_bia(p.attn.k, head * 12 + c) : pack_bia(p.attn.q, head * 12 + c) * qscale;
                else if (isk && c == 13) v = 1.0f;
            } else {
                const int k = j - G::V_B1, hid = 32 * (k >> 4) + rho(k & 15, hf);
                v = pack_bia(p.fc1, hid) * kLog2e;
            }
        } else {
            const int vch = i - 2 * G::VHF, head = vch >> 4, c = vch & 15;
            v = c < 12 ? pack_bia(p.attn.v, head * 12 + c) : (c == 12 ? 1.0f : 0.f);
        }
        vec[i] = v;
    }
    if (p.attn.bias_table) pack_rel_bias<false>(reinterpret_cast<float*>(dst + G::p_bias), p.attn.bias_table, a.ws, gtid, gsz);
}

struct L96 {
    static constexpr int C = 96, D = 12, HID_WIDE = 384, HID_NARROW = 192, PACK_GRID = 128, WAVES = 2;
    static constexpr const char *name = "win96", *pack_name = "pack_win96";
    template <int HID> using G = G96<HID>;
    template <int HID>
    static void pack(dim3 grid, const WinPackArgs& a, hipStream_t stream) { hipLaunchKernelGGL((pack96_kernel<HID>), grid, dim3(256), 0, stream, a); }
    template <int HID, int WS, int MODE, bool RAW>
    static int launch(const swf_block_desc& d, const WinArgs& a, int grid, hipStream_t stream) {
        if constexpr (MODE == WIN_BLOCK) {
            static const bool no_x8 = [] { const char* e = debug_env("SWF_WIN96X8"); return e && e[0] == '0'; }();
            if (!no_x8 && d.schedule != SWF_SCHED_THROUGHPUT && (a.H / WS) * (a.W / WS) <= 16) {
                constexpr int lds8 = (int)G96<HID>::l_total8;
                SWF_TRY((raise_lds_limit<&window96x8_kernel<HID, WS>>(lds8, "window96x8")));
                hipLaunchKernelGGL((window96x8_kernel<HID, WS>), dim3(std::min(grid, num_cus())), dim3(512), lds8, stream, a);
                return check_launch("window96x8");
            }
        }
        constexpr int lds = (int)G96<HID>::l_total;
        SWF_TRY((raise_lds_limit<&window96_kernel<HID, WS, MODE, RAW>>(lds, MODE == WIN_BLOCK ? "window96" : "window96 half")));
        hipLaunchKernelGGL((window96_kernel<HID, WS, MODE, RAW>), dim3(grid), dim3(256), lds, stream, a);
        return check_launch(MODE == WIN_BLOCK ? "window96" : "window96 (half block)");
    }
    template <int HID>
    static int launch16(const WinArgs& a, int nwin, hipStream_t stream) {
        constexpr int lds = (int)G96<HID>::l_total16;
        SWF_TRY(raise_lds_limit<&window96w16_kernel<HID>>(lds, "window96w16"));
        hipLaunchKernelGGL((window96w16_kernel<HID>), dim3(std::min(nwin, (num_cus() + 1) / 2), 2), dim3(256), lds, stream, a);
        return check_launch("window96w16");
    }
};

}

const WinLevel& win96_level() {
    static const WinLevel level = win_level<L96>();
    return level;
}

}

#ifdef W96_PROBE
extern "C" int swf_w96_probe_read(unsigned long long* out) {
    return hipMemcpyFromSymbol(out, HIP_SYMBOL(swf::w96_probe), 16 * sizeof(unsigned long long)) == hipSuccess ? 0 : 1;
}
#endif
```

swin_unet_image_fusion_amd/csrc/kernels_window.h:

```cpp
#pragma once
#include "win_level.h"

namespace swf {

bool window_block_supported(const swf_block_desc& d, int B, int H, int W);
size_t window_block_packed_bytes(const swf_block_desc& d);
bool window_block_out_of_place(const swf_block_desc& d);

int pack_window_block(const swf_block_desc& d, const swf_block_stream_params& px, const swf_block_stream_params& py,
                      void* packed_x, void* packed_y, hipStream_t stream);

int launch_window_block(const swf_block_desc& d, const void* packed_x, const void* packed_y,
                        const float* x_in, const float* y_in, float* x_out, float* y_out, int B, int H, int W,
                        hipStream_t stream, const void* next_packed_x = nullptr, const void* next_packed_y = nullptr,
                        size_t next_bytes = 0);

size_t window_half_packed_bytes(int C, int hid);
int pack_window_half(const swf_block_desc& d, const swf_block_stream_params& px, const swf_block_stream_params& py, char* pk,
                     size_t pb, hipStream_t stream);
int launch_window_half(const swf_block_desc& d, int mode, int raw, const char* pk, size_t pb, const float* x_in, const float* y_in,
                       float* x_out, float* y_out, int B, int H, int W, int ntok_x, int ntok_y, hipStream_t stream);

int launch_l2_warm(const void* p, size_t bytes, hipStream_t stream);

bool attn_core_mfma_supported(int wh, int ww, int head_dim);
int launch_attn_core_mfma(const float* const* Q, const float* const* K, const float* const* V, float* const* O,
                          const float* const* table, int nprob, int ldq, int ldk, int ldv, int ldo, int B, int H, int W,
                          int heads, int head_dim, int shift, hipStream_t stream, unsigned short* const* O_hi = nullptr,
                          unsigned short* const* O_lo = nullptr, const unsigned short* const* Q16 = nullptr,
                          const unsigned short* const* K16 = nullptr, const unsigned short* const* V16 = nullptr, int win = 8);

bool attn_core_mfma16_supported(int wh, int ww, int head_dim);
size_t attn_core_mfma16_scratch_floats(int nprob);
int launch_attn_core_mfma16(const float* const* Q, const float* const* K, const float* const* V, float* const* O,
                            const float* const* table, int nprob, int ldq, int ldk, int ldv, int ldo, int B, int H, int W,
                            int heads, int head_dim, int shift, float* bias_scratch, hipStream_t stream, unsigned short* const* O_hi = nullptr,
                            unsigned short* const* O_lo = nullptr, const unsigned short* const* Q16 = nullptr,
                            const unsigned short* const* K16 = nullptr, const unsigned short* const* V16 = nullptr);

}
```

swin_unet_image_fusion_amd/csrc/kernels_window.hip:

```cpp
#include "kernels_window.h"
#include "win_frag.h"

#include <algorithm>
#include <cstdlib>

namespace swf {

using namespace wf;

constexpr int cceil(int a, int b) { return (a + b - 1) / b; }
constexpr int cround(int a, int b) { return cceil(a, b) * b; }
constexpr size_t cmax(size_t a, size_t b) { return a > b ? a : b; }

struct AttnMfmaArgs {
    const float* Q[2]; const float* K[2]; const float* V[2]; float* O[2]; const float* table[2];
    unsigned short* Ohi[2]; unsigned short* Olo[2];
    const unsigned short* Q16[2]; const unsigned short* K16[2]; const unsigned short* V16[2];
    int ldq, ldk, ldv, ldo, B, H, W, heads, shift;
};

template <int D, int WS>
__global__ __launch_bounds__(128) void attn_core_mfma_kernel(AttnMfmaArgs a) {
    static_assert(WS == 7 || WS == 8, "window side");
    constexpr int T = 64, WH = WS, WW = WS, QS = cround(D, 8), QKS = cceil(D, 16), MT = cceil(D, 32), TW = 2 * WW - 1, VRS = T + 8;
// ... 464 lines not shown
}

bool attn_core_mfma16_supported(int wh, int ww, int head_dim) {
    return wh == 16 && ww == 16 && (head_dim == 3 || head_dim == 6 || head_dim == 12 || head_dim == 24 || head_dim == 48);
}

bool attn_core_mfma_supported(int wh, int ww, int head_dim) {
    return wh == ww && (wh == 8 || wh == 7) && (head_dim == 3 || head_dim == 6 || head_dim == 12 || head_dim == 24 || head_dim == 48);
}

int launch_attn_core_mfma(const float* const* Q, const float* const* K, const float* const* V, float* const* O,
                          const float* const* table, int nprob, int ldq, int ldk, int ldv, int ldo, int B, int H, int W,
                          int heads, int head_dim, int shift, hipStream_t stream, unsigned short* const* O_hi,
                          unsigned short* const* O_lo, const unsigned short* const* Q16, const unsigned short* const* K16,
                          const unsigned short* const* V16, int win) {
    AttnMfmaArgs a{};
    if ((win != 7 && win != 8) || H % win || W % win) return fail(SWF_ERR_UNSUPPORTED, "attn_core_mfma: window %d on a %d x %d map", win, H, W);
    if (Q16 && (head_dim % 4 || ldq % 4 || ldk % 4 || ldv % 4)) return fail(SWF_ERR_UNSUPPORTED, "attn_core_mfma: 16-bit operands need head_dim and strides %% 4 == 0");
    if (O_hi && head_dim % 4) return fail(SWF_ERR_UNSUPPORTED, "attn_core_mfma: split-plane output needs head_dim %% 4 == 0");
    for (int i = 0; i < nprob; ++i) {
        a.Q[i] = Q ? Q[i] : nullptr; a.K[i] = K ? K[i] : nullptr; a.V[i] = V ? V[i] : nullptr; a.O[i] = O ? O[i] : nullptr; a.table[i] = table[i];
        a.Q16[i] = Q16 ? Q16[i] : nullptr; a.K16[i] = Q16 ? K16[i] : nullptr; a.V16[i] = Q16 ? V16[i] : nullptr;
        a.Ohi[i] = O_hi ? O_hi[i] : nullptr; a.Olo[i] = O_hi ? O_lo[i] : nullptr;
    }
    a.ldq = ldq; a.ldk = ldk; a.ldv = ldv; a.ldo = ldo; a.B = B; a.H = H; a.W = W; a.heads = heads; a.shift = shift;
    switch (head_dim) {
        case 3: return launch_attn_mfma_t<3>(a, win, nprob, stream);
        case 6: return launch_attn_mfma_t<6>(a, win, nprob, stream);
        case 12: return launch_attn_mfma_t<12>(a, win, nprob, stream);
        case 24: return launch_attn_mfma_t<24>(a, win, nprob, stream);
        case 48: return launch_attn_mfma_t<48>(a, win, nprob, stream);
    }
    return fail(SWF_ERR_UNSUPPORTED, "attn_core_mfma: head_dim %d", head_dim);
}
static const WinLevel* level_of(int C) { return C == 24 ? &win24_level() : C == 48 ? &win48_level() : C == 96 ? &win96_level() : nullptr; }
static const WinLevel* level_of(const swf_block_desc& d) {
    const WinLevel* l = level_of(d.attn.channels);
    return l && l->supported(d) ? l : nullptr;
}

static int64_t image_bytes(const swf_block_desc& d, int H, int W) { return (int64_t)H * W * d.attn.channels * 4; }
constexpr int64_t kMaxLaunchBytes = (int64_t(1) << 31) - 1;

bool window_block_supported(const swf_block_desc& d, int B, int H, int W) {
    if (B <= 0 || H <= 0 || W <= 0 || !level_of(d)) return false;
    return H % d.attn.win_h == 0 && W % d.attn.win_w == 0 && image_bytes(d, H, W) <= kMaxLaunchBytes;
}

size_t window_block_packed_bytes(const swf_block_desc& d) {
    const WinLevel* l = level_of(d);
    return l ? l->packed_bytes(d) : 0;
}

bool window_block_out_of_place(const swf_block_desc& d) {
    return level_of(d) && d.attn.channels != 24 && d.attn.win_h == 16;
}

int pack_window_block(const swf_block_desc& d, const swf_block_stream_params& px, const swf_block_stream_params& py,
                      void* packed_x, void* packed_y, hipStream_t stream) {
    const WinLevel* l = level_of(d);
    if (!l) return fail(SWF_ERR_UNSUPPORTED, "pack_window_block: C=%d hidden=%d not covered", d.attn.channels, d.hidden);
    return l->pack(d, px, py, packed_x, packed_y, stream);
}

size_t window_half_packed_bytes(int C, int hid) {
    const WinLevel* l = level_of(C);
    return l ? l->half_packed_bytes(hid) : 0;
}

int pack_window_half(const swf_block_desc& d, const swf_block_stream_params& px, const swf_block_stream_params& py, char* pk,
                     size_t pb, hipStream_t stream) {
    const WinLevel* l = level_of(d.attn.channels);
    if (!l) return fail(SWF_ERR_UNSUPPORTED, "pack_window_half: C=%d not covered", d.attn.channels);
    return l->pack(d, px, py, pk, pk + pb, stream);
}

int launch_window_half(const swf_block_desc& d, int mode, int raw, const char* pk, size_t pb, const float* x_in, const float* y_in,
                       float* x_out, float* y_out, int B, int H, int W, int ntok_x, int ntok_y, hipStream_t stream) {
    const WinLevel* l = level_of(d.attn.channels);
    if (!l) return fail(SWF_ERR_UNSUPPORTED, "launch_window_half: C=%d not covered", d.attn.channels);
    return l->launch_half(d, mode, raw, pk, pk + pb, x_in, y_in, x_out, y_out, B, H, W, ntok_x, ntok_y, stream);
}

__global__ __launch_bounds__(256) void l2_warm_kernel(const char* __restrict__ p, int bytes, int* sink) {
    const int nsl = max(1, (int)gridDim.x / 8), sl = ((int)blockIdx.x / 8) % nsl;
    const int lines = (bytes + 127) / 128, per = (lines + nsl - 1) / nsl, l0 = sl * per, l1 = min(lines, l0 + per);
    unsigned acc = 0;
    for (int l = l0 + (int)threadIdx.x; l < l1; l += 256) acc ^= *reinterpret_cast<const unsigned*>(p + (size_t)l * 128);
    if (acc == 0x9e3779b9u && bytes < 0) *sink = 0;
}

int launch_l2_warm(const void* p, size_t bytes, hipStream_t stream) {
    if (!p || bytes == 0 || bytes > (1u << 30)) return SWF_OK;
    hipLaunchKernelGGL(l2_warm_kernel, dim3(256), dim3(256), 0, stream, static_cast<const char*>(p), (int)bytes, static_cast<int*>(nullptr));
    return check_launch("l2_warm");
}

int launch_window_block(const swf_block_desc& d, const void* packed_x, const void* packed_y, const float* x_in,
                        const float* y_in, float* x_out, float* y_out, int B, int H, int W, hipStream_t stream,
                        const void* next_packed_x, const void* next_packed_y, size_t next_bytes) {
    if (!window_block_supported(d, B, H, W))
        return fail(SWF_ERR_UNSUPPORTED, "window_block: C=%d hidden=%d, %d x %d map, window %d not covered", d.attn.channels, d.hidden, H, W, d.attn.win_h);
    const WinLevel* level = level_of(d);
    const int64_t img = image_bytes(d, H, W);
    const int per = (int)std::min<int64_t>(B, kMaxLaunchBytes / img);
    for (int b0 = 0; b0 < B; b0 += per) {
        const int nb = std::min(per, B - b0);
        const size_t off = (size_t)b0 * (size_t)(img / 4);
        const bool last = b0 + nb >= B;
        const void* nx = last ? next_packed_x : nullptr;
        const void* ny = last ? next_packed_y : nullptr;
        const int st = level->launch(d, packed_x, packed_y, x_in + off, y_in + off, x_out + off, y_out + off, nb, H, W, stream, nx, ny, next_bytes);
        if (st != SWF_OK) return st;
    }
    return SWF_OK;
}

}
```

swin_unet_image_fusion_amd/csrc/swf_api.hip:

```cpp
#include <algorithm>
#include <cmath>
#include <mutex>
#include <string>
#include <vector>

#include "kernels_generic.h"
#include <cstdlib>
#include "kernels_window.h"
#include "kernels_bwd.h"
#include "kernels_dropout.h"
#include "kernels_loss.h"
#include "kernels_optim.h"
#include "kernels_deep.h"
#include "kernels_patch.h"
#include "kernels_patchrr.h"
#include "kernels_deeppatch.h"
#include "kernels_mlp.h"
#include "kernels_qkvattn.h"
#include "kernels_attnproj.h"

namespace swf {

char* err_buf() {
    static thread_local char buf[512] = "";
// ... 376 lines not shown
    g2.scratch = b.sk; g2.scratch_floats = b.sk_floats;
    for (int s = 0; s < nstream; ++s)
        g2.p[s] = SpGemmProb{b.h_hi[s], b.h_lo[s], wv[s].w2_hi, wv[s].w2_lo, pp[s]->fc2.bias, xout[s], xout[s], nullptr, nullptr};
    return launch_gemm_sp(g2, nstream, (int)N, C, hid, C, SP_EPI_F32, stream);
}

static size_t block_packed_bytes(const swf_block_desc& d) {
    const size_t pb = window_block_packed_bytes(d);
    return pb ? pb : deep_block_packed_bytes(d);
}

static int check_block(const swf_block_desc* desc, const swf_block_stream_params* px, const swf_block_stream_params* py,
                       const float* x_in, const float* y_in, float* x_out, float* y_out, int B, int H, int W,
                       bool attn, bool mlp) {
    if (!desc) return fail(SWF_ERR_NULL, "desc is NULL");
    SWF_TRY(check_attn_desc(&desc->attn, B, H, W));
    if (mlp && desc->hidden <= 0) return fail(SWF_ERR_BAD_SHAPE, "hidden must be positive");
    SWF_TRY(check_stream_params(px, "x-stream", attn, mlp));
    if (!x_in || !x_out) return fail(SWF_ERR_NULL, "x tensors are NULL");
    if (py) {
        SWF_TRY(check_stream_params(py, "y-stream", attn, mlp));
        if (!y_in || !y_out) return fail(SWF_ERR_NULL, "y tensors are NULL with dual-path params");
    }
    return SWF_OK;
}

struct WindowBufs { char* packed; float *ox, *oy; };
static WindowBufs carve_window_block(Carver& ws, const swf_block_desc& d, int64_t N, bool prepacked, bool tmp_out) {
    WindowBufs b{};
    if (!prepacked) b.packed = reinterpret_cast<char*>(ws.floats((int64_t)(2 * window_block_packed_bytes(d) / 4)));
    if (tmp_out) {
        b.ox = ws.floats(2 * N * d.attn.channels);
        b.oy = b.ox ? b.ox + N * d.attn.channels : nullptr;
    }
    return b;
}
static size_t window_block_ws(const swf_block_desc& d, int B, int H, int W) {
    if (!window_block_supported(d, B, H, W)) return 0;
    size_t need = 0;
    for (int route = 0; route < 4; ++route) {
        if ((route & 2) && !window_block_out_of_place(d)) continue;
        Carver m = Carver::measure();
        carve_window_block(m, d, (int64_t)B * H * W, (route & 1) != 0, (route & 2) != 0);
        need = std::max(need, m.bytes());
    }
    return need;
}

static int basic_block_impl(const swf_block_desc* desc, const swf_block_stream_params* px,
                            const swf_block_stream_params* py, const float* x_in, const float* y_in, float* x_out,
                            float* y_out, int B, int H, int W, void* workspace, size_t workspace_bytes,
                            hipStream_t stream, const void* prepacked_x = nullptr, const void* prepacked_y = nullptr,
                            const void* next_x = nullptr, const void* next_y = nullptr, size_t next_bytes = 0,
                            const swf_block_stream_params* const* next_p = nullptr, bool* ln1_ready = nullptr) {
    if (desc->precision == SWF_PREC_FAST && py && window_block_supported(*desc, B, H, W)) {
        if (ln1_ready) *ln1_ready = false;
        const bool prepacked = prepacked_x && prepacked_y;
        const size_t pb = window_block_packed_bytes(*desc);
        const size_t map_bytes = (size_t)B * H * W * desc->attn.channels * 4;
        const bool via_tmp = window_block_out_of_place(*desc) && desc->cross && (x_in == x_out || y_in == y_out || x_in == y_out || y_in == x_out);
        Carver ws(workspace, workspace_bytes);
        const WindowBufs bufs = carve_window_block(ws, *desc, (int64_t)B * H * W, prepacked, via_tmp);
        if (!ws.ok()) return fail(SWF_ERR_WORKSPACE, "fused block workspace too small (need %zu B)", ws.bytes());
        char* w = bufs.packed;
        float *ox = via_tmp ? bufs.ox : x_out, *oy = via_tmp ? bufs.oy : y_out;
        if (prepacked) {
            SWF_TRY(launch_window_block(*desc, prepacked_x, prepacked_y, x_in, y_in, ox, oy, B, H, W, stream, next_x, next_y, next_bytes));
        } else {
            SWF_TRY(pack_window_block(*desc, *px, *py, w, w + pb, stream));
            SWF_TRY(launch_window_block(*desc, w, w + pb, x_in, y_in, ox, oy, B, H, W, stream));
        }
        if (via_tmp) {
            if (hipMemcpyAsync(x_out, ox, map_bytes, hipMemcpyDeviceToDevice, stream) != hipSuccess ||
                hipMemcpyAsync(y_out, oy, map_bytes, hipMemcpyDeviceToDevice, stream) != hipSuccess)
                return fail(SWF_ERR_HIP, "fused block: copy of the temporary outputs failed");
        }
        return SWF_OK;
    }
    auto aligned16 = [](const swf_block_stream_params* p) {
        if (!p) return true;
        const void* v[] = {p->ln1.gamma, p->ln1.beta, p->ln2.gamma, p->ln2.beta, p->attn.q.weight, p->attn.k.weight, p->attn.v.weight,
                           p->attn.proj.weight, p->fc1.weight, p->fc2.weight, p->attn.q.bias, p->attn.k.bias, p->attn.v.bias,
                           p->attn.proj.bias, p->fc1.bias, p->fc2.bias};
        uintptr_t bits = 0;
        for (const void* q : v) bits |= reinterpret_cast<uintptr_t>(q);
        return bits % 16 == 0;
    };
    const uintptr_t tbits = reinterpret_cast<uintptr_t>(x_in) | reinterpret_cast<uintptr_t>(y_in) | reinterpret_cast<uintptr_t>(x_out) |
                            reinterpret_cast<uintptr_t>(y_out);
    static const bool no_deep = debug_env("SWF_NO_DEEP") != nullptr;
    if (deep_block_supported(*desc) && !no_deep && tbits % 16 == 0 && aligned16(px) && aligned16(py)) {
        Carver ws(workspace, workspace_bytes);
        return deep_block_impl(desc, px, py, x_in, y_in, x_out, y_out, B, H, W, ws, stream, prepacked_x, prepacked_y, next_p, ln1_ready);
    }
    if (ln1_ready) *ln1_ready = false;
    {
        Carver ws(workspace, workspace_bytes);
        SWF_TRY(attn_halfblock_generic(desc, px, py, x_in, y_in, x_out, y_out, B, H, W, ws, stream));
    }
    Carver ws(workspace, workspace_bytes);
    return mlp_halfblock_generic(desc, px, py, x_out, y_out, x_out, y_out, B, H, W, ws, stream);
}

static int pad_amount(int len, int mult) { return (mult - len % mult) % mult; }

static int merge_shapes(int H, int W, int mh, int mw, int wh, int ww, int* Hm, int* Wm, int* Ho, int* Wo) {
    if (H <= 0 || W <= 0 || mh <= 0 || mw <= 0 || wh <= 0 || ww <= 0) return fail(SWF_ERR_BAD_SHAPE, "non-positive size");
    const int ph = pad_amount(H, mh), pw = pad_amount(W, mw);
    if (ph >= H || pw >= W) return fail(SWF_ERR_PAD, "reflect pad (%d,%d) >= map (%d,%d) before merging", ph, pw, H, W);
    *Hm = (H + ph) / mh;
    *Wm = (W + pw) / mw;
    const int qh = pad_amount(*Hm, wh), qw = pad_amount(*Wm, ww);
    if (qh >= *Hm || qw >= *Wm)
        return fail(SWF_ERR_PAD, "Padding size should be less than the corresponding input dimension: pad (%d,%d) on a %dx%d map",
                    qh, qw, *Hm, *Wm);
    *Ho = *Hm + qh;
    *Wo = *Wm + qw;
    return SWF_OK;
}

// ... 324 lines not shown
    const swf_model_desc* d = &canon;
    static std::mutex mu;
    static std::vector<ModelLayout*> cache;
    std::lock_guard<std::mutex> lock(mu);
    for (ModelLayout* l : cache)
        if (std::memcmp(&l->desc, d, sizeof(*d)) == 0) return l;
    ModelLayout* l = new ModelLayout();
    l->build(*d);
    cache.push_back(l);
    return l;
}

static swf_block_stream_params make_stream_params(const float* a, const BlockOff& o) {
    swf_block_stream_params p;
    p.ln1 = {a + o.ln1g, a + o.ln1b};
    p.attn.q = {a + o.wq, a + o.bq}; p.attn.k = {a + o.wk, a + o.bk}; p.attn.v = {a + o.wv, a + o.bv};
    p.attn.proj = {a + o.wp, a + o.bp}; p.attn.bias_table = a + o.table;
    p.ln2 = {a + o.ln2g, a + o.ln2b};
    p.fc1 = {a + o.w1, a + o.b1}; p.fc2 = {a + o.w2, a + o.b2};
    return p;
}

struct LevelShape { int Hin, Win, Hm, Wm, Ho, Wo; };

static int model_shapes(const swf_model_desc* d, int H, int W, LevelShape* ls) {
    int h = H, w = W;
    for (int s = 0; s < d->levels; ++s) {
        ls[s].Hin = h; ls[s].Win = w;
        SWF_TRY(merge_shapes(h, w, d->merge_h, d->merge_w, d->win_h, d->win_w, &ls[s].Hm, &ls[s].Wm, &ls[s].Ho, &ls[s].Wo));
        h = ls[s].Ho; w = ls[s].Wo;
    }
    if (d->head_ksize / 2 >= H || d->head_ksize / 2 >= W) return fail(SWF_ERR_PAD, "final conv reflect pad >= image");
    return SWF_OK;
}

static swf_block_desc level_block_desc(const swf_model_desc* d, int lvl, bool encoder) {
    swf_block_desc b;
    b.attn.channels = d->out_dims[lvl];
    b.attn.heads = d->heads;
    b.attn.head_dim = d->head_dim[lvl];
    b.attn.win_h = d->win_h; b.attn.win_w = d->win_w;
    b.attn.shift = 0;
    b.hidden = (encoder ? d->out_dims[lvl] : d->in_dims[lvl]) * d->mlp_ratio;
    b.cross = 0;
    b.precision = d->precision;
    b.schedule = d->schedule;
    return b;
}

static int block_pair4_impl(const swf_block_desc* desc, const swf_block_stream_params* px, const swf_block_stream_params* py,
                            const float* x_in, const float* y_in, float* x_out, float* y_out, int B, int H, int W,
                            void* workspace, size_t workspace_bytes, hipStream_t stream, const char* packed = nullptr,
                            const char* after = nullptr, size_t after_pb = 0, int32_t* equal_flags = nullptr,
                            const swf_block_stream_params* const* stage_next = nullptr, bool* ln1_io = nullptr) {
    const float* xi = x_in;
    const float* yi = y_in;
    const size_t pb = packed ? block_packed_bytes(*desc) : 0;
    bool ln1_ready = ln1_io ? *ln1_io : false;
    float *tx = nullptr, *ty = nullptr;
    size_t ws_left = workspace_bytes;
    {
        swf_block_desc dc = *desc;
        dc.cross = 1;
        if (desc->precision == SWF_PREC_FAST && py && window_block_supported(dc, B, H, W) && window_block_out_of_place(dc)) {
            Carver ws(workspace, workspace_bytes);
            const WindowBufs bufs = carve_window_block(ws, dc, (int64_t)B * H * W, packed != nullptr, true);
            if (workspace && ws.ok()) {
                tx = bufs.ox; ty = bufs.oy;
                ws_left = reinterpret_cast<char*>(tx) - static_cast<char*>(workspace);
            }
        }
    }
    for (int i = 0; i < 4; ++i) {
        swf_block_desc d = *desc;
        d.cross = i >= 2;
        d.attn.shift = i & 1;
        const void* pkx = (packed && pb) ? packed + (size_t)(2 * i) * pb : nullptr;
        const void* pky = (packed && pb) ? packed + (size_t)(2 * i + 1) * pb : nullptr;
        const void* nkx = (packed && pb && i < 3) ? packed + (size_t)(2 * i + 2) * pb : (i == 3 ? after : nullptr);
        const void* nky = (packed && pb && i < 3) ? packed + (size_t)(2 * i + 3) * pb : (i == 3 && after ? after + after_pb : nullptr);
        const swf_block_stream_params* nxt[2] = {i < 3 ? &px[i + 1] : nullptr, (i < 3 && py) ? &py[i + 1] : nullptr};
        const bool chain_out = i == 3 && stage_next && stage_next[0] && (!py || stage_next[1]);
        if (chain_out) { nxt[0] = stage_next[0]; nxt[1] = py ? stage_next[1] : nullptr; }
        if (equal_flags && d.cross && py)
            SWF_TRY(launch_all_equal(xi, yi, (int64_t)B * H * W * desc->attn.channels, equal_flags + (i - 2), stream));
        float* xo = (tx && i == 2) ? tx : x_out;
        float* yo = (tx && i == 2) ? ty : y_out;
        SWF_TRY(basic_block_impl(&d, &px[i], py ? &py[i] : nullptr, xi, yi, xo, yo, B, H, W, workspace, tx ? ws_left : workspace_bytes, stream, pkx, pky,
                                 nkx, nky, i == 3 ? after_pb : 0, (i < 3 || chain_out) ? nxt : nullptr, &ln1_ready));
        xi = xo; yi = yo;
    }
    if (ln1_io) *ln1_io = ln1_ready;
    return SWF_OK;
}

struct PackedPlan {
    size_t enc[SWF_MAX_LEVELS], dec[SWF_MAX_LEVELS], total;
    bool enc_on[SWF_MAX_LEVELS], dec_on[SWF_MAX_LEVELS];
    size_t penc[SWF_MAX_LEVELS], pdec[SWF_MAX_LEVELS], penc_b[SWF_MAX_LEVELS], pdec_b[SWF_MAX_LEVELS];
};
static PackedPlan packed_plan(const swf_model_desc* d) {
    PackedPlan p{};
    size_t off = 0;
    for (int s = 0; s < d->levels; ++s) {
        swf_block_desc be = level_block_desc(d, s, true);
        be.precision = SWF_PREC_FAST;
        const size_t pb = block_packed_bytes(be);
        p.enc_on[s] = pb > 0; p.enc[s] = off; off += 8 * pb;
    }
    for (int j = 0; j < d->levels; ++j) {
        swf_block_desc bd = level_block_desc(d, d->levels - 1 - j, false);
        bd.precision = SWF_PREC_FAST;
        const size_t pb = block_packed_bytes(bd);
        p.dec_on[j] = pb > 0; p.dec[j] = off; off += 8 * pb;
    }
    for (int s = 0; s < d->levels; ++s) {
        p.penc_b[s] = patch_image_bytes(0, d->in_dims[s], d->out_dims[s], d->merge_h, d->merge_w);
        p.penc[s] = off; off += 2 * p.penc_b[s];
    }
    for (int j = 0; j < d->levels; ++j) {
        const int lvl = d->levels - 1 - j;
        p.pdec_b[j] = patch_image_bytes(1, d->out_dims[lvl], d->in_dims[lvl], d->merge_h, d->merge_w);
        p.pdec[j] = off; off += 2 * p.pdec_b[j];
    }
    p.total = off;
    return p;
}

}

using namespace swf;

extern "C" {

int swf_version(void) { return SWF_VERSION_MAJOR * 1000 + SWF_VERSION_MINOR; }
const char* swf_last_error_string(void) { return err_buf(); }
const char* swf_status_string(int status) {
    switch (status) {
        case SWF_OK: return "ok";
        case SWF_ERR_NULL: return "null pointer";
        case SWF_ERR_BAD_SHAPE: return "bad shape";
        case SWF_ERR_PAD: return "reflect padding >= dimension";
        case SWF_ERR_UNSUPPORTED: return "unsupported configuration";
        case SWF_ERR_WORKSPACE: return "workspace too small";
        case SWF_ERR_HIP: return "HIP error";
        default: return "unknown status";
    }
}

static char* carve_window_half(Carver& ws, int C, int hid) { return reinterpret_cast<char*>(ws.floats((int64_t)(2 * window_half_packed_bytes(C, hid) / 4))); }
static char* window_half_images(void* workspace, size_t workspace_bytes, int C, int hid) {
    Carver ws(workspace, workspace_bytes);
    char* pk = carve_window_half(ws, C, hid);
    return ws.ok() ? pk : nullptr;
}
static size_t window_half_ws(int C, int hid) {
    Carver m = Carver::measure();
    carve_window_half(m, C, hid);
    return m.bytes();
}
static bool half_attn_shape(const swf_attn_desc& a, int H, int W) {
    return (a.channels == 24 || a.channels == 48 || a.channels == 96) && a.heads == 8 && a.head_dim * 8 == a.channels && a.win_h == a.win_w &&
           (a.win_h == 8 || a.win_h == 7) && H % a.win_h == 0 && W % a.win_w == 0;
}
static int half_attn_hidden(int C) { return 4 * C; }

static int mlp_half24(int C, int hid, int raw, const swf_block_stream_params* px, const swf_block_stream_params* py, const float* x_in,
                      const float* y_in, float* x_out, float* y_out, int64_t N, void* workspace, size_t workspace_bytes, hipStream_t stream) {
    const size_t pb = window_half_packed_bytes(C, hid);
    char* pk = window_half_images(workspace, workspace_bytes, C, hid);
    if (!pb || N <= 0 || N * C * 4 >= (int64_t(1) << 31) || !pk) return SWF_ERR_UNSUPPORTED;
    swf_block_desc bd{};
    bd.attn = swf_attn_desc{C, 8, C / 8, 8, 8, 0};
    bd.hidden = hid; bd.cross = 0; bd.precision = SWF_PREC_FAST;
    swf_block_stream_params sx = *px, sy = py ? *py : *px;
    sx.attn = swf_attn_params{}; sy.attn = swf_attn_params{};
// ... 686 lines not shown
    carve_model(m, desc, B, H, W, ls);
    return m.bytes();
}

size_t swf_model_packed_bytes(const swf_model_desc* desc) {
    if (check_model_desc(desc) != SWF_OK) return 0;
    return packed_plan(desc).total;
}

int swf_model_pack_weights(const swf_model_desc* desc, const float* arena, void* packed, size_t packed_bytes, swf_stream_t stream_) {
    SWF_TRY(check_model_desc(desc));
    if (!arena) return fail(SWF_ERR_NULL, "model_pack_weights: NULL arena");
    const PackedPlan plan = packed_plan(desc);
    if (plan.total == 0) return SWF_OK;
    if (!packed || packed_bytes < plan.total) return fail(SWF_ERR_WORKSPACE, "packed buffer too small (need %zu B)", plan.total);
    const ModelLayout* L = get_layout(desc);
    hipStream_t stream = as_stream(stream_);
    char* base = static_cast<char*>(packed);
    for (int pass = 0; pass < 2; ++pass)
        for (int k = 0; k < desc->levels; ++k) {
            const bool enc = pass == 0;
            if (!(enc ? plan.enc_on[k] : plan.dec_on[k])) continue;
            swf_block_desc bd = level_block_desc(desc, enc ? k : desc->levels - 1 - k, enc);
            bd.precision = SWF_PREC_FAST;
            const size_t pb = block_packed_bytes(bd);
            const bool fused = window_block_packed_bytes(bd) > 0;
            char* dst = base + (enc ? plan.enc[k] : plan.dec[k]);
            for (int i = 0; i < 4; ++i) {
                const swf_block_stream_params px = make_stream_params(arena, enc ? L->enc_blk[k][i][0] : L->dec_blk[k][i][0]);
                const swf_block_stream_params py = make_stream_params(arena, enc ? L->enc_blk[k][i][1] : L->dec_blk[k][i][1]);
                if (fused) {
                    SWF_TRY(pack_window_block(bd, px, py, dst + (size_t)(2 * i) * pb, dst + (size_t)(2 * i + 1) * pb, stream));
                } else {
                    SWF_TRY(pack_deep_block(bd, px, dst + (size_t)(2 * i) * pb, stream));
                    SWF_TRY(pack_deep_block(bd, py, dst + (size_t)(2 * i + 1) * pb, stream));
                }
            }
        }
    for (int k = 0; k < desc->levels; ++k) {
        const int lvl = desc->levels - 1 - k;
        for (int st = 0; st < 2; ++st) {
            if (plan.penc_b[k]) {
                const PatchOff& o = L->enc_patch[k][st];
                SWF_TRY(pack_patch_image(0, desc->in_dims[k], desc->out_dims[k], desc->merge_h, desc->merge_w,
                                         swf_patch_params{{arena + o.w, arena + o.b}, {arena + o.g, arena + o.bt}},
                                         base + plan.penc[k] + st * plan.penc_b[k], stream));
            }
            if (plan.pdec_b[k]) {
                const PatchOff& o = L->dec_patch[k][st];
                SWF_TRY(pack_patch_image(1, desc->out_dims[lvl], desc->in_dims[lvl], desc->merge_h, desc->merge_w,
                                         swf_patch_params{{arena + o.w, arena + o.b}, {arena + o.g, arena + o.bt}},
                                         base + plan.pdec[k] + st * plan.pdec_b[k], stream));
            }
        }
    }
    return SWF_OK;
}

static int model_forward_impl(const swf_model_desc* desc, const float* arena, const char* packed, const float* ir, const float* vis, float* out,
                              int32_t B, int32_t H, int32_t W, void* workspace, size_t workspace_bytes, swf_stream_t stream_,
                              int32_t* equal_flags = nullptr, hipEvent_t* marks = nullptr) {
    SWF_TRY(check_model_desc(desc));
    const PackedPlan plan = packed_plan(desc);
    if (!arena || !ir || !vis || !out) return fail(SWF_ERR_NULL, "model_forward: NULL tensor");
    if (B <= 0) return fail(SWF_ERR_BAD_SHAPE, "model_forward: empty batch");
    LevelShape ls[SWF_MAX_LEVELS];
    SWF_TRY(model_shapes(desc, H, W, ls));
    const ModelLayout* L = get_layout(desc);
    hipStream_t stream = as_stream(stream_);
    const int n = desc->levels;
    Carver ws(workspace, workspace_bytes);
    const ModelBufs bufs = carve_model(ws, desc, B, H, W, ls);
    if (!workspace || !ws.ok()) return fail(SWF_ERR_WORKSPACE, "model workspace too small: have %zu B, need %zu B", workspace_bytes, ws.bytes());

    auto patch_params = [&](const PatchOff& o) { return swf_patch_params{{arena + o.w, arena + o.b}, {arena + o.g, arena + o.bt}}; };

    int nmark = 0;
    auto mark = [&]() -> int {
        if (marks && hipEventRecord(marks[nmark++], stream) != hipSuccess) return fail(SWF_ERR_HIP, "model_forward: hipEventRecord failed");
        return SWF_OK;
    };
    SWF_TRY(mark());
    const float* cur[2] = {ir, vis};
    bool ln1_carry = false;
    swf_block_stream_params dpx0 = make_stream_params(arena, L->dec_blk[0][0][0]), dpy0 = make_stream_params(arena, L->dec_blk[0][0][1]);
    const swf_block_stream_params* dec_first[2] = {&dpx0, &dpy0};
    for (int s = 0; s < n; ++s) {
        swf_patch_params pm[2] = {patch_params(L->enc_patch[s][0]), patch_params(L->enc_patch[s][1])};
        const swf_patch_params* pmp[2] = {&pm[0], &pm[1]};
        const void* prr_enc[2] = {packed ? packed + plan.penc[s] : nullptr, packed ? packed + plan.penc[s] + plan.penc_b[s] : nullptr};
        swf_block_stream_params px[4], py[4];
        for (int i = 0; i < 4; ++i) { px[i] = make_stream_params(arena, L->enc_blk[s][i][0]); py[i] = make_stream_params(arena, L->enc_blk[s][i][1]); }
        swf_block_desc bd = level_block_desc(desc, s, true);
        const swf_block_stream_params* first_blk[2] = {&px[0], &py[0]};
        const bool deep_stage = packed && desc->precision == SWF_PREC_FAST && window_block_packed_bytes(bd) == 0 && deep_block_supported(bd);
        ln1_carry = false;
        SWF_TRY(patch_merge_impl(pmp, 2, cur, bufs.act[s], B, ls[s].Hin, ls[s].Win, desc->in_dims[s], desc->out_dims[s], desc->merge_h,
                                 desc->merge_w, desc->win_h, desc->win_w, bufs.scratch, bufs.scratch_bytes, stream, desc->precision == SWF_PREC_FAST,
                                 (packed && plan.penc_b[s]) ? prr_enc : nullptr, deep_stage ? first_blk : nullptr, deep_stage ? &ln1_carry : nullptr));
        SWF_TRY(mark());
        const char* after = nullptr;
        size_t after_pb = 0;
        if (packed && s + 1 < n) {
            swf_block_desc nb = level_block_desc(desc, s + 1, true);
            if (window_block_packed_bytes(nb) && plan.enc_on[s + 1]) { after = packed + plan.enc[s + 1]; after_pb = window_block_packed_bytes(nb); }
        }
        const bool chain = deep_stage && s == n - 1;
        SWF_TRY(block_pair4_impl(&bd, px, py, bufs.act[s][0], bufs.act[s][1], bufs.act[s][0], bufs.act[s][1], B, ls[s].Ho, ls[s].Wo, bufs.scratch, bufs.scratch_bytes, stream,
                                 (packed && plan.enc_on[s]) ? packed + plan.enc[s] : nullptr, after, after_pb,
                                 equal_flags ? equal_flags + 2 * s : nullptr, chain ? dec_first : nullptr, deep_stage ? &ln1_carry : nullptr));
        if (!chain) ln1_carry = false;
        SWF_TRY(mark());
        cur[0] = bufs.act[s][0]; cur[1] = bufs.act[s][1];
    }
    for (int j = 0; j < n; ++j) {
        const int lvl = n - 1 - j;
        swf_block_stream_params px[4], py[4];
        for (int i = 0; i < 4; ++i) { px[i] = make_stream_params(arena, L->dec_blk[j][i][0]); py[i] = make_stream_params(arena, L->dec_blk[j][i][1]); }
        swf_block_desc bd = level_block_desc(desc, lvl, false);
        const char* after = nullptr;
        size_t after_pb = 0;
        if (packed && j + 1 < n) {
            swf_block_desc nb = level_block_desc(desc, n - 2 - j, false);
            if (window_block_packed_bytes(nb) && plan.dec_on[j + 1]) { after = packed + plan.dec[j + 1]; after_pb = window_block_packed_bytes(nb); }
        }
        bool ln1_in = ln1_carry;
        SWF_TRY(block_pair4_impl(&bd, px, py, bufs.act[lvl][0], bufs.act[lvl][1], bufs.act[lvl][0], bufs.act[lvl][1], B, ls[lvl].Ho, ls[lvl].Wo, bufs.scratch, bufs.scratch_bytes, stream,
                                 (packed && plan.dec_on[j]) ? packed + plan.dec[j] : nullptr, after, after_pb,
                                 equal_flags ? equal_flags + 2 * (n + j) : nullptr, nullptr, &ln1_in));
        SWF_TRY(mark());
        const bool warm_next = after && window_block_packed_bytes(bd) == 0;
        bool warmed = false;
        swf_block_stream_params npx0{}, npy0{};
        bool next_deep = false;
        if (packed && desc->precision == SWF_PREC_FAST && j + 1 < n) {
            swf_block_desc nb = level_block_desc(desc, n - 2 - j, false);
            nb.precision = SWF_PREC_FAST;
            next_deep = window_block_packed_bytes(nb) == 0 && deep_block_supported(nb);
            if (next_deep) { npx0 = make_stream_params(arena, L->dec_blk[j + 1][0][0]); npy0 = make_stream_params(arena, L->dec_blk[j + 1][0][1]); }
        }
        const swf_block_stream_params* next_first[2] = {&npx0, &npy0};
        ln1_carry = false;
        swf_patch_params pm[2] = {patch_params(L->dec_patch[j][0]), patch_params(L->dec_patch[j][1])};
        const swf_patch_params* pmp[2] = {&pm[0], &pm[1]};
        const float* ins[2] = {bufs.act[lvl][0], bufs.act[lvl][1]};
        const float* skip[2] = {lvl > 0 ? bufs.act[lvl - 1][0] : nullptr, lvl > 0 ? bufs.act[lvl - 1][1] : nullptr};
        float* outs[2] = {lvl > 0 ? bufs.act[lvl - 1][0] : bufs.full[0], lvl > 0 ? bufs.act[lvl - 1][1] : bufs.full[1]};
        const void* prr_dec[2] = {packed ? packed + plan.pdec[j] : nullptr, packed ? packed + plan.pdec[j] + plan.pdec_b[j] : nullptr};
        SWF_TRY(patch_unmerge_impl(pmp, 2, ins, lvl > 0 ? skip : nullptr, outs, B, ls[lvl].Ho, ls[lvl].Wo, ls[lvl].Hm, ls[lvl].Wm,
                                   desc->out_dims[lvl], desc->in_dims[lvl], desc->merge_h, desc->merge_w, ls[lvl].Hin, ls[lvl].Win,
                                   bufs.scratch, bufs.scratch_bytes, stream, desc->precision == SWF_PREC_FAST, (packed && plan.pdec_b[j]) ? prr_dec : nullptr,
                                   warm_next ? after : nullptr, warm_next ? after_pb : 0, &warmed, next_deep ? next_first : nullptr,
                                   next_deep ? &ln1_carry : nullptr));
        if (warm_next && !warmed) SWF_TRY(launch_l2_warm(after, 2 * after_pb, stream));
        SWF_TRY(mark());
    }
    swf_head_params hp{arena + L->h_c1w, arena + L->h_c1b, arena + L->h_g, arena + L->h_b, arena + L->h_m, arena + L->h_v,
                       arena + L->h_c2w, arena + L->h_c2b};
    Carver hw(bufs.scratch, bufs.scratch_bytes);
    float* tmp = carve_head_fwd(hw, B, H, W);
    SWF_TRY(launch_head(bufs.full[0], bufs.full[1], tmp, out, hp, B, H, W, desc->head_ksize, stream));
    return mark();
}

int swf_model_forward(const swf_model_desc* desc, const float* arena, const float* ir, const float* vis, float* out,
                      int32_t B, int32_t H, int32_t W, void* workspace, size_t workspace_bytes, swf_stream_t stream) {
    return model_forward_impl(desc, arena, nullptr, ir, vis, out, B, H, W, workspace, workspace_bytes, stream);
}

int swf_model_forward_packed(const swf_model_desc* desc, const float* arena, const void* packed, const float* ir, const float* vis,
                             float* out, int32_t B, int32_t H, int32_t W, void* workspace, size_t workspace_bytes, swf_stream_t stream) {
    return model_forward_impl(desc, arena, static_cast<const char*>(packed), ir, vis, out, B, H, W, workspace, workspace_bytes, stream);
}

int swf_model_forward_checked(const swf_model_desc* desc, const float* arena, const void* packed, const float* ir, const float* vis,
                              float* out, int32_t B, int32_t H, int32_t W, void* workspace, size_t workspace_bytes,
                              int32_t* cross_equal_flags, swf_stream_t stream) {
    if (!cross_equal_flags) return fail(SWF_ERR_NULL, "model_forward_checked: NULL flags");
    if (check_model_desc(desc) != SWF_OK) return SWF_ERR_BAD_SHAPE;
    hipError_t e = hipMemsetD32Async(reinterpret_cast<hipDeviceptr_t>(cross_equal_flags), 1, (size_t)4 * desc->levels, as_stream(stream));
    if (e != hipSuccess) return fail(SWF_ERR_HIP, "model_forward_checked: memset: %s", hipGetErrorString(e));
    return model_forward_impl(desc, arena, static_cast<const char*>(packed), ir, vis, out, B, H, W, workspace, workspace_bytes, stream,
                              cross_equal_flags);
}

int swf_model_forward_profiled(const swf_model_desc* desc, const float* arena, const void* packed, const float* ir, const float* vis,
                               float* out, int32_t B, int32_t H, int32_t W, void* workspace, size_t workspace_bytes, float* seg_ms,
                               int32_t seg_count, swf_stream_t stream) {
    if (!seg_ms) return fail(SWF_ERR_NULL, "model_forward_profiled: NULL seg_ms");
    if (check_model_desc(desc) != SWF_OK) return SWF_ERR_BAD_SHAPE;
    const int nseg = 4 * desc->levels + 1;
    if (seg_count < nseg) return fail(SWF_ERR_BAD_SHAPE, "model_forward_profiled: seg_ms holds %d values, need %d", seg_count, nseg);
    hipEvent_t ev[4 * SWF_MAX_LEVELS + 2];
    int made = 0, st = SWF_OK;
    for (; made < nseg + 1; ++made)
        if (hipEventCreate(&ev[made]) != hipSuccess) { st = fail(SWF_ERR_HIP, "model_forward_profiled: hipEventCreate failed"); break; }
    if (st == SWF_OK)
        st = model_forward_impl(desc, arena, static_cast<const char*>(packed), ir, vis, out, B, H, W, workspace, workspace_bytes, stream, nullptr, ev);
    if (st == SWF_OK && hipStreamSynchronize(as_stream(stream)) != hipSuccess) st = fail(SWF_ERR_HIP, "model_forward_profiled: synchronize failed");
    for (int i = 0; st == SWF_OK && i < nseg; ++i)
        if (hipEventElapsedTime(&seg_ms[i], ev[i], ev[i + 1]) != hipSuccess) st = fail(SWF_ERR_HIP, "model_forward_profiled: hipEventElapsedTime failed");
    for (int i = 0; i < made; ++i) (void)hipEventDestroy(ev[i]);
    return st;
}

int swf_tensors_equal(const float* a, const float* b, int64_t count, int32_t* flag, swf_stream_t stream) {
    if (!flag) return fail(SWF_ERR_NULL, "tensors_equal: NULL flag");
    hipError_t e = hipMemsetD32Async(reinterpret_cast<hipDeviceptr_t>(flag), 1, 1, as_stream(stream));
    if (e != hipSuccess) return fail(SWF_ERR_HIP, "tensors_equal: memset: %s", hipGetErrorString(e));
    return launch_all_equal(a, b, count, flag, as_stream(stream));
}

static int check_fusion_loss(const swf_loss_desc* desc, int32_t B, int32_t H, int32_t W) {
    if (!desc) return fail(SWF_ERR_NULL, "fusion_loss: NULL descriptor");
    if (B <= 0 || H <= 0 || W <= 0) return fail(SWF_ERR_BAD_SHAPE, "fusion_loss: empty tensor (B=%d H=%d W=%d)", B, H, W);
    if (desc->ssim_mode != 0 && desc->ssim_mode != 1)
        return fail(SWF_ERR_UNSUPPORTED, "fusion_loss: ssim_mode %d (0 = MS-SSIM + L1, 1 = single-scale SSIM)", desc->ssim_mode);
    if (desc->ssim_mode == 1 && (H < 6 || W < 6))
        return fail(SWF_ERR_PAD, "fusion_loss: the 11-tap SSIM window reflects 5 pixels, the map is %dx%d", H, W);
    return SWF_OK;
}

size_t swf_fusion_loss_workspace_bytes(const swf_loss_desc* desc, int32_t B, int32_t H, int32_t W, int32_t with_grad) {
    if (check_fusion_loss(desc, B, H, W) != SWF_OK) return 0;
    return fusion_loss_workspace_bytes(*desc, B, H, W, with_grad != 0);
}

int swf_fusion_loss(const swf_loss_desc* desc, const float* fusion, const float* ir, const float* vis, float* terms, float* grad_fusion,
                    int32_t B, int32_t H, int32_t W, void* workspace, size_t workspace_bytes, swf_stream_t stream) {
    if (!desc || !fusion || !ir || !vis || !terms) return fail(SWF_ERR_NULL, "fusion_loss: NULL descriptor, image or terms");
    SWF_TRY(check_fusion_loss(desc, B, H, W));
    const size_t need = fusion_loss_workspace_bytes(*desc, B, H, W, grad_fusion != nullptr);
    if (!workspace || workspace_bytes < need)
        return fail(SWF_ERR_WORKSPACE, "fusion_loss: workspace of %zu bytes, %zu needed", workspace ? workspace_bytes : (size_t)0, need);
    return fusion_loss(*desc, fusion, ir, vis, terms, grad_fusion, B, H, W, workspace, workspace_bytes, as_stream(stream));
}
// ... 121 lines not shown
```

swin_unet_image_fusion_amd/csrc/win_host.h:

```cpp
#pragma once
#include "win_frag.h"
#include "win_level.h"

#include <algorithm>

namespace swf {
namespace {

__host__ __device__ constexpr int kslot(int s, int hf, int e) { return 32 * (s >> 1) + wf::rho(8 * (s & 1) + e, hf); }

__device__ __forceinline__ float pack_wgt(const swf_linear& l, int i) { return l.weight ? l.weight[i] : 0.f; }
__device__ __forceinline__ float pack_bia(const swf_linear& l, int n) { return (l.weight && l.bias) ? l.bias[n] : 0.f; }

template <bool LANE_MAJOR>
__device__ __forceinline__ void pack_rel_bias(float* bm, const float* table, int ws, int gtid, int gsz) {
    const int ktb = ws == 16 ? 0 : 1;
    for (int i = gtid; i < (ws == 16 ? 15 : 4) * 1024; i += gsz) {
        const int outer = i >> (10 + ktb);
        const int reg = LANE_MAJOR ? i & 15 : 4 * ((i >> 8) & 3) + (i & 3);
        const int kt = ((LANE_MAJOR ? i >> 4 : i >> 10)) & ((1 << ktb) - 1);
        const int lane = (LANE_MAJOR ? i >> (4 + ktb) : i >> 2) & 63;
        const int key = 32 * kt + wf::rho(reg, lane >> 5), q = lane & 31;
        if (ws == 16) {
            const int dy = 2 * (outer - 7) + (key >> 4) - (q >> 4), dx = (key & 15) - (q & 15);
// ... 40 lines not shown
    if (d.hidden == L::HID_WIDE) L::template pack<L::HID_WIDE>(dim3(L::PACK_GRID, 2), a, stream);
    else L::template pack<L::HID_NARROW>(dim3(L::PACK_GRID, 2), a, stream);
    return check_launch(L::pack_name);
}

template <class L> bool win_rows_fit(int64_t tokens) { return tokens * L::C * 4 < (int64_t(1) << 31); }

inline WinArgs win_args(const swf_block_desc& d, const void* packed_x, const void* packed_y, const float* x_in, const float* y_in,
                        float* x_out, float* y_out, int B, int H, int W) {
    WinArgs a{};
    a.in[0] = x_in; a.in[1] = y_in; a.out[0] = x_out; a.out[1] = y_out;
    a.packed[0] = static_cast<const char*>(packed_x); a.packed[1] = static_cast<const char*>(packed_y);
    a.B = B; a.H = H; a.W = W; a.shift = d.attn.shift; a.cross = d.cross;
    return a;
}

template <class L, int HID, int MODE, bool RAW>
int win_launch_ws(const swf_block_desc& d, const WinArgs& a, int grid, hipStream_t stream) {
    if constexpr (MODE != WIN_MLP) {
        if (d.attn.win_h != 8) return L::template launch<HID, 7, MODE, RAW>(d, a, grid, stream);
    }
    return L::template launch<HID, 8, MODE, RAW>(d, a, grid, stream);
}
template <class L, int MODE, bool RAW>
int win_launch_as(const swf_block_desc& d, const WinArgs& a, int nwin, hipStream_t stream) {
    const int grid = std::min(nwin, L::WAVES * num_cus());
    if constexpr (MODE != WIN_ATTN) {
        if (d.hidden != L::HID_WIDE) return win_launch_ws<L, L::HID_NARROW, MODE, RAW>(d, a, grid, stream);
    }
    return win_launch_ws<L, L::HID_WIDE, MODE, RAW>(d, a, grid, stream);
}

template <class L>
int win_launch_half(const swf_block_desc& d, int mode, int raw, const void* packed_x, const void* packed_y, const float* x_in,
                    const float* y_in, float* x_out, float* y_out, int B, int H, int W, int ntok_x, int ntok_y, hipStream_t stream) {
    const int wsd = d.attn.win_h;
    if (mode != WIN_ATTN && mode != WIN_MLP) return fail(SWF_ERR_UNSUPPORTED, "%s_half: mode %d", L::name, mode);
    if (d.attn.channels != L::C || !win_hidden_ok<L>(d.hidden)) return fail(SWF_ERR_UNSUPPORTED, "%s_half: shape not covered", L::name);
    WinArgs a = win_args(d, packed_x, packed_y, x_in, y_in, x_out, y_out, B, H, W);
    a.ntok[0] = ntok_x; a.ntok[1] = ntok_y;
    if (mode == WIN_ATTN) {
        if (!win_supported<L>(d) || wsd == 16 || H % wsd || W % wsd) return fail(SWF_ERR_UNSUPPORTED, "%s_half: shape not covered", L::name);
        if (!win_rows_fit<L>((int64_t)B * H * W)) return fail(SWF_ERR_UNSUPPORTED, "%s_half: map exceeds the 2 GB buffer window", L::name);
        const int nwin = B * (H / wsd) * (W / wsd);
        return raw ? win_launch_as<L, WIN_ATTN, true>(d, a, nwin, stream) : win_launch_as<L, WIN_ATTN, false>(d, a, nwin, stream);
    }
    const int ntok = std::max(ntok_x, ntok_y);
    if (!win_rows_fit<L>(ntok) || ntok_x <= 0) return fail(SWF_ERR_UNSUPPORTED, "%s_half: token count", L::name);
    const int nwin = (ntok + 63) / 64;
    return raw ? win_launch_as<L, WIN_MLP, true>(d, a, nwin, stream) : win_launch_as<L, WIN_MLP, false>(d, a, nwin, stream);
}

template <class L>
int win_launch(const swf_block_desc& d, const void* packed_x, const void* packed_y, const float* x_in, const float* y_in,
               float* x_out, float* y_out, int B, int H, int W, hipStream_t stream, const void* next_packed_x,
               const void* next_packed_y, size_t next_bytes) {
    const int wsd = d.attn.win_h;
    if (!win_supported<L>(d) || H % wsd || W % wsd) return fail(SWF_ERR_UNSUPPORTED, "%s: shape not covered", L::name);
    if (!win_rows_fit<L>((int64_t)B * H * W))
        return fail(SWF_ERR_UNSUPPORTED, "%s: a stream of %d x %d x %d tokens exceeds the 2 GB buffer window", L::name, B, H, W);
    WinArgs a = win_args(d, packed_x, packed_y, x_in, y_in, x_out, y_out, B, H, W);
    a.warm[0] = static_cast<const char*>(next_packed_x); a.warm[1] = static_cast<const char*>(next_packed_y);
    if (!a.warm[1]) a.warm[0] = nullptr;
    a.warm_bytes = (int)(next_bytes ? next_bytes : win_packed_bytes<L>(d));
    const int nwin = B * (H / wsd) * (W / wsd);
    if (wsd != 16) return win_launch_as<L, WIN_BLOCK, false>(d, a, nwin, stream);
    return d.hidden == L::HID_WIDE ? L::template launch16<L::HID_WIDE>(a, nwin, stream) : L::template launch16<L::HID_NARROW>(a, nwin, stream);
}

template <class L>
constexpr WinLevel win_level() {
    return {win_supported<L>, win_packed_bytes<L>, win_half_packed_bytes<L>, win_pack<L>, win_launch_half<L>, win_launch<L>};
}

}
}
```

swin_unet_image_fusion_amd/csrc/win_level.h:

```cpp
#pragma once
#include "swf_common.h"

namespace swf {

struct WinArgs {
    const float* in[2];
    float* out[2];
    const char* packed[2];
    const char* warm[2];
    int B, H, W, shift, cross, warm_bytes;
    int ntok[2];
};

constexpr int WIN_BLOCK = 0, WIN_ATTN = 1, WIN_MLP = 2;

struct WinPackArgs {
    swf_block_stream_params p[2];
    char* dst[2];
    int ws;
};

struct WinLevel {
    bool (*supported)(const swf_block_desc& d);
    size_t (*packed_bytes)(const swf_block_desc& d);
    size_t (*half_packed_bytes)(int hidden);
    int (*pack)(const swf_block_desc& d, const swf_block_stream_params& px, const swf_block_stream_params& py, void* packed_x,
                void* packed_y, hipStream_t stream);
    int (*launch_half)(const swf_block_desc& d, int mode, int raw, const void* packed_x, const void* packed_y, const float* x_in,
                       const float* y_in, float* x_out, float* y_out, int B, int H, int W, int ntok_x, int ntok_y, hipStream_t stream);
    int (*launch)(const swf_block_desc& d, const void* packed_x, const void* packed_y, const float* x_in, const float* y_in,
                  float* x_out, float* y_out, int B, int H, int W, hipStream_t stream, const void* next_packed_x,
                  const void* next_packed_y, size_t next_bytes);
};

const WinLevel& win24_level();
const WinLevel& win48_level();
const WinLevel& win96_level();

}
```

Measured before the change: 8973 pairs/s.

## Fuse decoder patch-unmerge tail into the window-block kernels at levels 24 and 48

Adds an optional tail stage to the C=24 and C=48 window-attention block kernels. After the block, the kernel computes the 2x2 patch-unmerge projection with MFMA, applies LayerNorm and ELU, adds the skip connection and writes the upsampled output directly. It also adds packing for the tail weights in the matching fragment order, plus a host query saying which levels can take the tail. The goal is to avoid writing and re-reading the block output at full resolution and to save a separate patch-expand launch. In exchange the kernel uses more LDS and registers, which may reduce occupancy.

```diff
diff --git a/include/swinfuse.h b/include/swinfuse.h
--- a/include/swinfuse.h
+++ b/include/swinfuse.h
@@ -283,6 +283,7 @@
 int swf_model_forward_checked(const swf_model_desc* desc, const float* arena, const void* packed,
                               const float* ir, const float* vis, float* out, int32_t B, int32_t H, int32_t W,
                               void* workspace, size_t workspace_bytes, int32_t* cross_equal_flags, swf_stream_t stream);
+int32_t swf_model_unmerge_tail_mask(const swf_model_desc* desc, int32_t B, int32_t H, int32_t W);
 int swf_model_forward_profiled(const swf_model_desc* desc, const float* arena, const void* packed,
                                const float* ir, const float* vis, float* out, int32_t B, int32_t H, int32_t W,
                                void* workspace, size_t workspace_bytes, float* seg_ms, int32_t seg_count, swf_stream_t stream);
diff --git a/swin_unet_image_fusion_amd/_lib.py b/swin_unet_image_fusion_amd/_lib.py
--- a/swin_unet_image_fusion_amd/_lib.py
+++ b/swin_unet_image_fusion_amd/_lib.py
@@ -178,6 +178,7 @@
     "swf_model_pack_weights": (C.c_int, [P(ModelDesc), _vp, _vp, _sz, _vp]),
     "swf_model_forward_packed": (C.c_int, [P(ModelDesc), _vp, _vp, _vp, _vp, _vp, _i32, _i32, _i32, _vp, _sz, _vp]),
     "swf_model_forward_checked": (C.c_int, [P(ModelDesc), _vp, _vp, _vp, _vp, _vp, _i32, _i32, _i32, _vp, _sz, _vp, _vp]),
+    "swf_model_unmerge_tail_mask": (_i32, [P(ModelDesc), _i32, _i32, _i32]),
     "swf_model_forward_profiled": (C.c_int, [P(ModelDesc), _vp, _vp, _vp, _vp, _vp, _i32, _i32, _i32, _vp, _sz, P(C.c_float), _i32, _vp]),
     "swf_tensors_equal": (C.c_int, [_vp, _vp, _i64, _vp, _vp]),
     "swf_fusion_loss_workspace_bytes": (_sz, [P(LossDesc), _i32, _i32, _i32, _i32]),
diff --git a/swin_unet_image_fusion_amd/csrc/kernels_patchrr.h b/swin_unet_image_fusion_amd/csrc/kernels_patchrr.h
--- a/swin_unet_image_fusion_amd/csrc/kernels_patchrr.h
+++ b/swin_unet_image_fusion_amd/csrc/kernels_patchrr.h
@@ -7,6 +7,9 @@
 size_t patch_rr_packed_bytes(int decoder, int Cin, int Cout, int mh, int mw);
 int pack_patch_rr(int decoder, int Cin, int Cout, int mh, int mw, const float* weight, const float* bias, const float* gamma,
                   const float* beta, void* dst, hipStream_t stream);
+size_t unmerge_tail_packed_bytes(int Cin, int Cout);
+int pack_unmerge_tail(int Cin, int Cout, const float* weight, const float* bias, const float* gamma, const float* beta, void* dst,
+                      hipStream_t stream);
 int launch_patch_rr(const PatchFusedDesc& d, const void* const* packed, int nstream, hipStream_t stream);
 
 }
diff --git a/swin_unet_image_fusion_amd/csrc/kernels_patchrr.hip b/swin_unet_image_fusion_amd/csrc/kernels_patchrr.hip
--- a/swin_unet_image_fusion_amd/csrc/kernels_patchrr.hip
+++ b/swin_unet_image_fusion_amd/csrc/kernels_patchrr.hip
@@ -234,7 +234,7 @@
     }
 }
 
-struct PrrPackArgs { const float* w; const float* bias; const float* gamma; const float* beta; char* dst; int K, N; };
+struct PrrPackArgs { const float* w; const float* bias; const float* gamma; const float* beta; char* dst; int K, N, acc_k; };
 
 template <int KS, int NT>
 __global__ __launch_bounds__(256) void patch_rr_pack_kernel(PrrPackArgs a) {
@@ -243,7 +243,7 @@
     for (int idx = gtid; idx < P::NFRAG * 512; idx += gsz) {
         const int f = idx >> 9, lane = (idx >> 3) & 63, e = idx & 7, r = lane & 31, hf = lane >> 5;
         const int hl = f & 1, ks = (f >> 1) % KS, nt = f / (2 * KS);
-        const int n = 32 * nt + r, k = 16 * ks + 8 * hf + e;
+        const int n = 32 * nt + r, k = a.acc_k ? 32 * (ks >> 1) + rho(8 * (ks & 1) + e, hf) : 16 * ks + 8 * hf + e;
         const float val = (n < a.N && k < a.K) ? a.w[(int64_t)n * a.K + k] : 0.f;
         const bf16 hi = (bf16)val;
         reinterpret_cast<bf16*>(a.dst)[idx] = hl ? (bf16)(val - (float)hi) : hi;
@@ -297,11 +297,28 @@
                   const float* beta, void* dst, hipStream_t stream) {
     int ks, nt;
     if (!shape_class(decoder, Cin, Cout, mh, mw, &ks, &nt)) return fail(SWF_ERR_UNSUPPORTED, "pack_patch_rr: shape not covered");
-    PrrPackArgs a{weight, bias, gamma, beta, static_cast<char*>(dst), decoder ? Cin : 4 * Cin, decoder ? 4 * Cout : Cout};
+    PrrPackArgs a{weight, bias, gamma, beta, static_cast<char*>(dst), decoder ? Cin : 4 * Cin, decoder ? 4 * Cout : Cout, 0};
 #define SWF_PRR_PACK(KS_, NT_) if (ks == KS_ && nt == NT_) { hipLaunchKernelGGL((patch_rr_pack_kernel<KS_, NT_>), dim3(32), dim3(256), 0, stream, a); return check_launch("pack_patch_rr"); }
     SWF_PRR_PACK(1, 1) SWF_PRR_PACK(2, 1) SWF_PRR_PACK(3, 3) SWF_PRR_PACK(6, 2) SWF_PRR_PACK(6, 6) SWF_PRR_PACK(12, 3)
 #undef SWF_PRR_PACK
     return fail(SWF_ERR_UNSUPPORTED, "pack_patch_rr: shape class");
+}
+
+size_t unmerge_tail_packed_bytes(int Cin, int Cout) {
+    int ks, nt;
+    const bool ok = (Cin == 24 && Cout == 1) || (Cin == 48 && Cout == 24);
+    return ok && shape_class(1, Cin, Cout, 2, 2, &ks, &nt) ? patch_rr_packed_bytes(1, Cin, Cout, 2, 2) : 0;
+}
+
+int pack_unmerge_tail(int Cin, int Cout, const float* weight, const float* bias, const float* gamma, const float* beta, void* dst,
+                      hipStream_t stream) {
+    int ks, nt;
+    if (!unmerge_tail_packed_bytes(Cin, Cout) || !shape_class(1, Cin, Cout, 2, 2, &ks, &nt)) return fail(SWF_ERR_UNSUPPORTED, "pack_unmerge_tail: shape not covered");
+    PrrPackArgs a{weight, bias, gamma, beta, static_cast<char*>(dst), Cin, 4 * Cout, 1};
+#define SWF_TAIL_PACK(KS_, NT_) if (ks == KS_ && nt == NT_) { hipLaunchKernelGGL((patch_rr_pack_kernel<KS_, NT_>), dim3(32), dim3(256), 0, stream, a); return check_launch("pack_unmerge_tail"); }
+    SWF_TAIL_PACK(2, 1) SWF_TAIL_PACK(3, 3)
+#undef SWF_TAIL_PACK
+    return fail(SWF_ERR_UNSUPPORTED, "pack_unmerge_tail: shape class");
 }
 
 int launch_patch_rr(const PatchFusedDesc& d, const void* const* packed, int nstream, hipStream_t stream) {
diff --git a/swin_unet_image_fusion_amd/csrc/kernels_win24.hip b/swin_unet_image_fusion_amd/csrc/kernels_win24.hip
--- a/swin_unet_image_fusion_amd/csrc/kernels_win24.hip
+++ b/swin_unet_image_fusion_amd/csrc/kernels_win24.hip
@@ -1,4 +1,5 @@
 #include "win_host.h"
+#include "win_tail.h"
 
 namespace swf {
 namespace {
@@ -6,6 +7,8 @@
 using namespace wf;
 
 constexpr int W24_WAVES = 3;
+constexpr int W24_TAIL_COUT = 1;
+using T24 = WinTailG<24, W24_TAIL_COUT>;
 
 template <int HID_>
 struct G24 {
@@ -155,14 +158,15 @@
 }
 
 
-template <int HID, int WS, int MODE = WIN_BLOCK, bool RAW = false>
+template <int HID, int WS, int MODE = WIN_BLOCK, bool RAW = false, int TAIL = WIN_TAIL_NONE>
 __global__ __launch_bounds__(256, W24_WAVES) void window24_kernel(WinArgs args) {
     using G = G24<HID>;
     static_assert(WS == 7 || WS == 8, "window side");
     static_assert(MODE == WIN_BLOCK || MODE == WIN_ATTN || MODE == WIN_MLP, "mode");
     static_assert(!RAW || MODE != WIN_BLOCK, "RAW belongs to the half-block modes");
+    static_assert(TAIL == WIN_TAIL_NONE || MODE == WIN_BLOCK, "the tail follows a whole block");
     constexpr bool ATT = MODE != WIN_MLP, MLP = MODE != WIN_ATTN;
-    __shared__ __attribute__((aligned(16))) char smem[G::l_total];
+    __shared__ __attribute__((aligned(16))) char smem[G::l_total + (TAIL ? T24::LDS_FLOATS * 4 : 0)];
     u32x4* kimg = reinterpret_cast<u32x4*>(smem + G::l_k);
     u32x4* vimg = reinterpret_cast<u32x4*>(smem + G::l_v);
     float* lvec = reinterpret_cast<float*>(smem + G::l_vec);
@@ -175,6 +179,7 @@
     const int kvs = args.cross ? 1 - ws : ws;
 
     for (int i = tid; i < 2 * 2 * 64; i += 256) lvec[i] = reinterpret_cast<const float*>(args.packed[i >> 7] + G::p_vec)[i & 127];
+    if constexpr (TAIL) tail_fill_vectors<T24>(reinterpret_cast<float*>(smem + G::l_total), args.tail, tid);
     const __amdgpu_buffer_rsrc_t wrs = __builtin_amdgcn_make_buffer_rsrc(const_cast<char*>(uniform_ptr(args.packed[ws])), 0, (int)G::p_total, 0x00020000);
     const __amdgpu_buffer_rsrc_t krs = __builtin_amdgcn_make_buffer_rsrc(const_cast<char*>(uniform_ptr(args.packed[kvs])), 0, (int)G::p_total, 0x00020000);
     const int act_bytes = ATT ? args.B * H * W * 24 * 4 : args.ntok[ws] * 24 * 4;
@@ -199,6 +204,7 @@
     if constexpr (ATT) load_bias();
     const bool half1 = hf != 0;
     const bool col_masked = half1 != (((r >> 2) & 1) != 0);
+    const int ws_s = TAIL ? __builtin_amdgcn_readfirstlane(ws) : 0;
     __syncthreads();
 
     int it = 0;
@@ -324,7 +330,18 @@
             }
         }
 
-        store_rows24(ors, tokoff, res);
+        if constexpr (TAIL) {
+            u32x4 tw[T24::NFRAG];
+            tail_request<T24>(args.tail, ws_s, lane_w, tw);
+            float n[16];
+#pragma unroll
+            for (int i = 0; i < 16; ++i) n[i] = i < 12 ? res[i] : 0.f;
+            const bool live = (WS == 8 || (ty < WS && tx < WS)) && (int)oy < args.tail.Hm && (int)ox < args.tail.Wm;
+            unmerge_tail<T24, W24_TAIL_COUT>(args.tail, ws_s, reinterpret_cast<const float*>(smem + G::l_total) + ws_s * (T24::LDS_FLOATS / 2), tw, n, b,
+                                             (int)oy, (int)ox, live, lane_w, args.B * args.tail.Ho * args.tail.Wo * W24_TAIL_COUT * 4);
+        } else {
+            store_rows24(ors, tokoff, res);
+        }
     }
 
     if (args.warm[0]) warm_next_block<256>(args, tid);
@@ -554,9 +571,10 @@
     template <int HID> using G = G24<HID>;
     template <int HID>
     static void pack(dim3 grid, const WinPackArgs& a, hipStream_t stream) { hipLaunchKernelGGL((pack24_kernel<HID>), grid, dim3(256), 0, stream, a); }
-    template <int HID, int WS, int MODE, bool RAW>
+    static constexpr int TAIL_COUT = W24_TAIL_COUT;
+    template <int HID, int WS, int MODE, bool RAW, int TAIL = WIN_TAIL_NONE>
     static int launch(const swf_block_desc&, const WinArgs& a, int grid, hipStream_t stream) {
-        hipLaunchKernelGGL((window24_kernel<HID, WS, MODE, RAW>), dim3(grid), dim3(256), 0, stream, a);
+        hipLaunchKernelGGL((window24_kernel<HID, WS, MODE, RAW, TAIL>), dim3(grid), dim3(256), 0, stream, a);
         return check_launch(MODE == WIN_BLOCK ? "window24" : "window24 (half block)");
     }
     template <int HID>
diff --git a/swin_unet_image_fusion_amd/csrc/kernels_win48.hip b/swin_unet_image_fusion_amd/csrc/kernels_win48.hip
--- a/swin_unet_image_fusion_amd/csrc/kernels_win48.hip
+++ b/swin_unet_image_fusion_amd/csrc/kernels_win48.hip
@@ -1,4 +1,5 @@
 #include "win_host.h"
+#include "win_tail.h"
 
 namespace swf {
 namespace {
@@ -6,6 +7,8 @@
 using namespace wf;
 
 constexpr int W48_WAVES = 2;
+constexpr int W48_TAIL_COUT = 24;
+using T48 = WinTailG<48, W48_TAIL_COUT>;
 
 template <int HID_>
 struct G48 {
@@ -124,13 +127,14 @@
     }
 }
 
-template <int HID, int WS, int MODE = WIN_BLOCK, bool RAW = false>
+template <int HID, int WS, int MODE = WIN_BLOCK, bool RAW = false, int TAIL = WIN_TAIL_NONE>
 __global__ __launch_bounds__(256, W48_WAVES) void window48_kernel(WinArgs args) {
     using G = G48<HID>;
     static_assert(WS == 7 || WS == 8, "window side");
     static_assert(!RAW || MODE != WIN_BLOCK, "RAW belongs to the half-block modes");
+    static_assert(TAIL == WIN_TAIL_NONE || MODE == WIN_BLOCK, "the tail follows a whole block");
     constexpr bool ATT = MODE != WIN_MLP, MLP = MODE != WIN_ATTN;
-    __shared__ __attribute__((aligned(16))) char smem[G::l_total];
+    __shared__ __attribute__((aligned(16))) char smem[G::l_total + (TAIL ? T48::LDS_FLOATS * 4 : 0)];
     u32x4* kimg = reinterpret_cast<u32x4*>(smem + G::l_k);
     u32x4* vimg = reinterpret_cast<u32x4*>(smem + G::l_v);
     float* lvec = reinterpret_cast<float*>(smem + G::l_vec);
@@ -156,6 +160,7 @@
     const bool half1 = hf != 0;
     const bool col_masked = half1 != (((r >> 2) & 1) != 0);
     const f32x16 zero16 = {0.f, 0.f, 0.f, 0.f, 0.f, 0.f, 0.f, 0.f, 0.f, 0.f, 0.f, 0.f, 0.f, 0.f, 0.f, 0.f};
+    const int ws_s = TAIL ? __builtin_amdgcn_readfirstlane(ws) : 0;
 
     for (int win = blockIdx.x; win < nwin; win += gridDim.x) {
         SWF_WF_FENCE();
@@ -200,6 +205,7 @@
             if (win == (int)blockIdx.x) {
                 static_assert(G::VSTREAM % 4 == 0 && G::p_vec % 16 == 0, "vector sections move as 16-byte groups");
                     fill_vectors<G::VSTREAM / 4, 256>(lvec, args.packed[0] + G::p_vec, args.packed[1] + G::p_vec, tid);
+                if constexpr (TAIL) tail_fill_vectors<T48>(reinterpret_cast<float*>(smem + G::l_total), args.tail, tid);
                 __syncthreads();
             }
             u32x4 xh[3], xl[3];
@@ -302,6 +308,8 @@
             }
         }
 
+        u32x4 tw[TAIL ? T48::NFRAG : 1];
+
         if constexpr (MLP) {
             u32x4 w1[2][6];
             auto req1 = [&](int tI, u32x4 (&dst)[6]) {
@@ -327,6 +335,9 @@
             for (int tI = 0; tI < G::NT1; ++tI) {
                 SWF_WF_FENCE();
                 if (tI + 1 < G::NT1) { req1(tI + 1, w1[(tI + 1) & 1]); req2(tI + 1, w2[(tI + 1) & 1]); }
+                if constexpr (TAIL) {
+                    if (tI == G::NT1 - 1) tail_request<T48>(args.tail, ws_s, lane, tw);
+                }
                 SWF_WF_FENCE();
                 const u32x4 (&w)[6] = w1[tI & 1];
                 f32x16 acc = zero16;
@@ -351,11 +362,20 @@
             }
         }
 
+        if constexpr (TAIL) {
+            float n[24];
+#pragma unroll
+            for (int i = 0; i < 24; ++i) n[i] = i < 16 ? res0[i] : res1[i - 16];
+            const bool live = (WS == 8 || (ty < WS && tx < WS)) && oy < args.tail.Hm && ox < args.tail.Wm;
+            unmerge_tail<T48, W48_TAIL_COUT>(args.tail, ws_s, reinterpret_cast<const float*>(smem + G::l_total) + ws_s * (T48::LDS_FLOATS / 2), tw, n, b,
+                                             oy, ox, live, lane, args.B * args.tail.Ho * args.tail.Wo * W48_TAIL_COUT * 4);
+        } else {
 #pragma unroll
         for (int a = 0; a < 6; ++a) {
             const f32x4 v = a < 4 ? f32x4{res0[4 * a], res0[4 * a + 1], res0[4 * a + 2], res0[4 * a + 3]}
                                   : f32x4{res1[4 * (a - 4)], res1[4 * (a - 4) + 1], res1[4 * (a - 4) + 2], res1[4 * (a - 4) + 3]};
             __builtin_amdgcn_raw_buffer_store_b128(__builtin_bit_cast(u32x4, v), ors, tokoff, 32 * a, 0);
+        }
         }
     }
 
@@ -660,9 +680,10 @@
     template <int HID> using G = G48<HID>;
     template <int HID>
     static void pack(dim3 grid, const WinPackArgs& a, hipStream_t stream) { hipLaunchKernelGGL((pack48_kernel<HID>), grid, dim3(256), 0, stream, a); }
-    template <int HID, int WS, int MODE, bool RAW>
+    static constexpr int TAIL_COUT = W48_TAIL_COUT;
+    template <int HID, int WS, int MODE, bool RAW, int TAIL = WIN_TAIL_NONE>
     static int launch(const swf_block_desc&, const WinArgs& a, int grid, hipStream_t stream) {
-        hipLaunchKernelGGL((window48_kernel<HID, WS, MODE, RAW>), dim3(grid), dim3(256), 0, stream, a);
+        hipLaunchKernelGGL((window48_kernel<HID, WS, MODE, RAW, TAIL>), dim3(grid), dim3(256), 0, stream, a);
         return check_launch(MODE == WIN_BLOCK ? "window48" : "window48 (half block)");
     }
     template <int HID>
diff --git a/swin_unet_image_fusion_amd/csrc/kernels_win96.hip b/swin_unet_image_fusion_amd/csrc/kernels_win96.hip
--- a/swin_unet_image_fusion_amd/csrc/kernels_win96.hip
+++ b/swin_unet_image_fusion_amd/csrc/kernels_win96.hip
@@ -1011,6 +1011,7 @@
     template <int HID> using G = G96<HID>;
     template <int HID>
     static void pack(dim3 grid, const WinPackArgs& a, hipStream_t stream) { hipLaunchKernelGGL((pack96_kernel<HID>), grid, dim3(256), 0, stream, a); }
+    static constexpr int TAIL_COUT = 0;
     template <int HID, int WS, int MODE, bool RAW>
     static int launch(const swf_block_desc& d, const WinArgs& a, int grid, hipStream_t stream) {
         if constexpr (MODE == WIN_BLOCK) {
diff --git a/swin_unet_image_fusion_amd/csrc/kernels_window.h b/swin_unet_image_fusion_amd/csrc/kernels_window.h
--- a/swin_unet_image_fusion_amd/csrc/kernels_window.h
+++ b/swin_unet_image_fusion_amd/csrc/kernels_window.h
@@ -13,7 +13,9 @@
 int launch_window_block(const swf_block_desc& d, const void* packed_x, const void* packed_y,
                         const float* x_in, const float* y_in, float* x_out, float* y_out, int B, int H, int W,
                         hipStream_t stream, const void* next_packed_x = nullptr, const void* next_packed_y = nullptr,
-                        size_t next_bytes = 0);
+                        size_t next_bytes = 0, const WinTail* tail = nullptr);
+
+int window_block_tail_cout(const swf_block_desc& d, int B, int H, int W);
 
 size_t window_half_packed_bytes(int C, int hid);
 int pack_window_half(const swf_block_desc& d, const swf_block_stream_params& px, const swf_block_stream_params& py, char* pk,
diff --git a/swin_unet_image_fusion_amd/csrc/kernels_window.hip b/swin_unet_image_fusion_amd/csrc/kernels_window.hip
--- a/swin_unet_image_fusion_amd/csrc/kernels_window.hip
+++ b/swin_unet_image_fusion_amd/csrc/kernels_window.hip
@@ -540,6 +540,11 @@
     return l ? l->packed_bytes(d) : 0;
 }
 
+int window_block_tail_cout(const swf_block_desc& d, int B, int H, int W) {
+    if (!window_block_supported(d, B, H, W)) return 0;
+    return level_of(d)->tail_cout(d, H, W);
+}
+
 bool window_block_out_of_place(const swf_block_desc& d) {
     return level_of(d) && d.attn.channels != 24 && d.attn.win_h == 16;
 }
@@ -586,19 +591,31 @@
 
 int launch_window_block(const swf_block_desc& d, const void* packed_x, const void* packed_y, const float* x_in,
                         const float* y_in, float* x_out, float* y_out, int B, int H, int W, hipStream_t stream,
-                        const void* next_packed_x, const void* next_packed_y, size_t next_bytes) {
+                        const void* next_packed_x, const void* next_packed_y, size_t next_bytes, const WinTail* tail) {
     if (!window_block_supported(d, B, H, W))
         return fail(SWF_ERR_UNSUPPORTED, "window_block: C=%d hidden=%d, %d x %d map, window %d not covered", d.attn.channels, d.hidden, H, W, d.attn.win_h);
     const WinLevel* level = level_of(d);
     const int64_t img = image_bytes(d, H, W);
-    const int per = (int)std::min<int64_t>(B, kMaxLaunchBytes / img);
+    int per = (int)std::min<int64_t>(B, kMaxLaunchBytes / img);
+    if (tail) {
+        const int64_t timg = (int64_t)tail->Ho * tail->Wo * level->tail_cout(d, H, W) * 4;
+        if (timg <= 0 || timg > kMaxLaunchBytes) return fail(SWF_ERR_UNSUPPORTED, "window_block: un-merged map of one image exceeds the 2 GB buffer window");
+        per = (int)std::min<int64_t>(per, kMaxLaunchBytes / timg);
+    }
     for (int b0 = 0; b0 < B; b0 += per) {
         const int nb = std::min(per, B - b0);
         const size_t off = (size_t)b0 * (size_t)(img / 4);
         const bool last = b0 + nb >= B;
         const void* nx = last ? next_packed_x : nullptr;
         const void* ny = last ? next_packed_y : nullptr;
-        const int st = level->launch(d, packed_x, packed_y, x_in + off, y_in + off, x_out + off, y_out + off, nb, H, W, stream, nx, ny, next_bytes);
+        WinTail ts{};
+        if (tail) {
+            ts = *tail;
+            const size_t toff = (size_t)b0 * tail->Ho * tail->Wo * level->tail_cout(d, H, W);
+            for (int s = 0; s < 2; ++s) { ts.out[s] += toff; if (ts.skip[s]) ts.skip[s] += toff; }
+        }
+        const int st = level->launch(d, packed_x, packed_y, x_in + off, y_in + off, tail ? nullptr : x_out + off, tail ? nullptr : y_out + off, nb, H, W, stream,
+                                     nx, ny, next_bytes, tail ? &ts : nullptr);
         if (st != SWF_OK) return st;
     }
     return SWF_OK;
diff --git a/swin_unet_image_fusion_amd/csrc/swf_api.hip b/swin_unet_image_fusion_amd/csrc/swf_api.hip
--- a/swin_unet_image_fusion_amd/csrc/swf_api.hip
+++ b/swin_unet_image_fusion_amd/csrc/swf_api.hip
@@ -452,7 +452,10 @@
                             float* y_out, int B, int H, int W, void* workspace, size_t workspace_bytes,
                             hipStream_t stream, const void* prepacked_x = nullptr, const void* prepacked_y = nullptr,
                             const void* next_x = nullptr, const void* next_y = nullptr, size_t next_bytes = 0,
-                            const swf_block_stream_params* const* next_p = nullptr, bool* ln1_ready = nullptr) {
+                            const swf_block_stream_params* const* next_p = nullptr, bool* ln1_ready = nullptr,
+                            const WinTail* tail = nullptr) {
+    if (tail && !(desc->precision == SWF_PREC_FAST && py && prepacked_x && prepacked_y && window_block_tail_cout(*desc, B, H, W)))
+        return fail(SWF_ERR_UNSUPPORTED, "basic_block: un-merge tail on a block that does not run the pre-packed fused kernel");
     if (desc->precision == SWF_PREC_FAST && py && window_block_supported(*desc, B, H, W)) {
         if (ln1_ready) *ln1_ready = false;
         const bool prepacked = prepacked_x && prepacked_y;
@@ -465,7 +468,7 @@
         char* w = bufs.packed;
         float *ox = via_tmp ? bufs.ox : x_out, *oy = via_tmp ? bufs.oy : y_out;
         if (prepacked) {
-            SWF_TRY(launch_window_block(*desc, prepacked_x, prepacked_y, x_in, y_in, ox, oy, B, H, W, stream, next_x, next_y, next_bytes));
+            SWF_TRY(launch_window_block(*desc, prepacked_x, prepacked_y, x_in, y_in, ox, oy, B, H, W, stream, next_x, next_y, next_bytes, tail));
         } else {
             SWF_TRY(pack_window_block(*desc, *px, *py, w, w + pb, stream));
             SWF_TRY(launch_window_block(*desc, w, w + pb, x_in, y_in, ox, oy, B, H, W, stream));
@@ -896,7 +899,8 @@
                             const float* x_in, const float* y_in, float* x_out, float* y_out, int B, int H, int W,
                             void* workspace, size_t workspace_bytes, hipStream_t stream, const char* packed = nullptr,
                             const char* after = nullptr, size_t after_pb = 0, int32_t* equal_flags = nullptr,
-                            const swf_block_stream_params* const* stage_next = nullptr, bool* ln1_io = nullptr) {
+                            const swf_block_stream_params* const* stage_next = nullptr, bool* ln1_io = nullptr,
+                            const WinTail* tail = nullptr) {
     const float* xi = x_in;
     const float* yi = y_in;
     const size_t pb = packed ? block_packed_bytes(*desc) : 0;
@@ -931,7 +935,7 @@
         float* xo = (tx && i == 2) ? tx : x_out;
         float* yo = (tx && i == 2) ? ty : y_out;
         SWF_TRY(basic_block_impl(&d, &px[i], py ? &py[i] : nullptr, xi, yi, xo, yo, B, H, W, workspace, tx ? ws_left : workspace_bytes, stream, pkx, pky,
-                                 nkx, nky, i == 3 ? after_pb : 0, (i < 3 || chain_out) ? nxt : nullptr, &ln1_ready));
+                                 nkx, nky, i == 3 ? after_pb : 0, (i < 3 || chain_out) ? nxt : nullptr, &ln1_ready, i == 3 ? tail : nullptr));
         xi = xo; yi = yo;
     }
     if (ln1_io) *ln1_io = ln1_ready;
@@ -942,7 +946,15 @@
     size_t enc[SWF_MAX_LEVELS], dec[SWF_MAX_LEVELS], total;
     bool enc_on[SWF_MAX_LEVELS], dec_on[SWF_MAX_LEVELS];
     size_t penc[SWF_MAX_LEVELS], pdec[SWF_MAX_LEVELS], penc_b[SWF_MAX_LEVELS], pdec_b[SWF_MAX_LEVELS];
+    size_t ptail[SWF_MAX_LEVELS], ptail_b[SWF_MAX_LEVELS];
 };
+static size_t tail_image_bytes(const swf_model_desc* d, int lvl) {
+    swf_block_desc bd = level_block_desc(d, lvl, false);
+    bd.precision = SWF_PREC_FAST;
+    if (!window_block_packed_bytes(bd) || bd.attn.win_h == 16 || d->merge_h != 2 || d->merge_w != 2) return 0;
+    if (!patch_rr_supported(1, d->out_dims[lvl], d->in_dims[lvl], d->merge_h, d->merge_w)) return 0;
+    return unmerge_tail_packed_bytes(d->out_dims[lvl], d->in_dims[lvl]);
+}
 static PackedPlan packed_plan(const swf_model_desc* d) {
     PackedPlan p{};
     size_t off = 0;
@@ -966,6 +978,10 @@
         const int lvl = d->levels - 1 - j;
         p.pdec_b[j] = patch_image_bytes(1, d->out_dims[lvl], d->in_dims[lvl], d->merge_h, d->merge_w);
         p.pdec[j] = off; off += 2 * p.pdec_b[j];
+    }
+    for (int j = 0; j < d->levels; ++j) {
+        p.ptail_b[j] = tail_image_bytes(d, d->levels - 1 - j);
+        p.ptail[j] = off; off += 2 * p.ptail_b[j];
     }
     p.total = off;
     return p;
@@ -1758,9 +1774,24 @@
                                          swf_patch_params{{arena + o.w, arena + o.b}, {arena + o.g, arena + o.bt}},
                                          base + plan.pdec[k] + st * plan.pdec_b[k], stream));
             }
+            if (plan.ptail_b[k]) {
+                const PatchOff& o = L->dec_patch[k][st];
+                SWF_TRY(pack_unmerge_tail(desc->out_dims[lvl], desc->in_dims[lvl], arena + o.w, arena + o.b, arena + o.g, arena + o.bt,
+                                          base + plan.ptail[k] + st * plan.ptail_b[k], stream));
+            }
         }
     }
     return SWF_OK;
+}
+
+static bool unmerge_tail_fused(const swf_model_desc* desc, const PackedPlan& plan, const LevelShape* ls, int j, int B) {
+    static const bool no_tail = [] { const char* e = debug_env("SWF_FUSE_UNMERGE"); return e && e[0] == '0'; }();
+    static const bool no_prr_dec = debug_env("SWF_NO_FUSED_PATCH") != nullptr || debug_env("SWF_NO_PATCH_RR") != nullptr;
+    const int lvl = desc->levels - 1 - j;
+    if (desc->precision != SWF_PREC_FAST || no_tail || no_prr_dec || !plan.dec_on[j] || !plan.pdec_b[j] || !plan.ptail_b[j]) return false;
+    const swf_block_desc bd = level_block_desc(desc, lvl, false);
+    return window_block_tail_cout(bd, B, ls[lvl].Ho, ls[lvl].Wo) == desc->in_dims[lvl] &&
+           (int64_t)ls[lvl].Hin * ls[lvl].Win * desc->in_dims[lvl] * 4 < (int64_t(1) << 31);
 }
 
 static int model_forward_impl(const swf_model_desc* desc, const float* arena, const char* packed, const float* ir, const float* vis, float* out,
@@ -1831,10 +1862,23 @@
             if (window_block_packed_bytes(nb) && plan.dec_on[j + 1]) { after = packed + plan.dec[j + 1]; after_pb = window_block_packed_bytes(nb); }
         }
         bool ln1_in = ln1_carry;
+        const float* skip[2] = {lvl > 0 ? bufs.act[lvl - 1][0] : nullptr, lvl > 0 ? bufs.act[lvl - 1][1] : nullptr};
+        float* outs[2] = {lvl > 0 ? bufs.act[lvl - 1][0] : bufs.full[0], lvl > 0 ? bufs.act[lvl - 1][1] : bufs.full[1]};
+        const bool fuse_tail = packed && !marks && unmerge_tail_fused(desc, plan, ls, j, B);
+        WinTail tail{};
+        if (fuse_tail) {
+            for (int t = 0; t < 2; ++t) { tail.out[t] = outs[t]; tail.skip[t] = skip[t]; tail.packed[t] = packed + plan.ptail[j] + t * plan.ptail_b[j]; }
+            tail.Hm = ls[lvl].Hm; tail.Wm = ls[lvl].Wm; tail.Ho = ls[lvl].Hin; tail.Wo = ls[lvl].Win;
+        }
         SWF_TRY(block_pair4_impl(&bd, px, py, bufs.act[lvl][0], bufs.act[lvl][1], bufs.act[lvl][0], bufs.act[lvl][1], B, ls[lvl].Ho, ls[lvl].Wo, bufs.scratch, bufs.scratch_bytes, stream,
                                  (packed && plan.dec_on[j]) ? packed + plan.dec[j] : nullptr, after, after_pb,
-                                 equal_flags ? equal_flags + 2 * (n + j) : nullptr, nullptr, &ln1_in));
+                                 equal_flags ? equal_flags + 2 * (n + j) : nullptr, nullptr, &ln1_in, fuse_tail ? &tail : nullptr));
         SWF_TRY(mark());
+        if (fuse_tail) {
+            ln1_carry = false;
+            SWF_TRY(mark());
+            continue;
+        }
         const bool warm_next = after && window_block_packed_bytes(bd) == 0;
         bool warmed = false;
         swf_block_stream_params npx0{}, npy0{};
@@ -1850,8 +1894,6 @@
         swf_patch_params pm[2] = {patch_params(L->dec_patch[j][0]), patch_params(L->dec_patch[j][1])};
         const swf_patch_params* pmp[2] = {&pm[0], &pm[1]};
         const float* ins[2] = {bufs.act[lvl][0], bufs.act[lvl][1]};
-        const float* skip[2] = {lvl > 0 ? bufs.act[lvl - 1][0] : nullptr, lvl > 0 ? bufs.act[lvl - 1][1] : nullptr};
-        float* outs[2] = {lvl > 0 ? bufs.act[lvl - 1][0] : bufs.full[0], lvl > 0 ? bufs.act[lvl - 1][1] : bufs.full[1]};
         const void* prr_dec[2] = {packed ? packed + plan.pdec[j] : nullptr, packed ? packed + plan.pdec[j] + plan.pdec_b[j] : nullptr};
         SWF_TRY(patch_unmerge_impl(pmp, 2, ins, lvl > 0 ? skip : nullptr, outs, B, ls[lvl].Ho, ls[lvl].Wo, ls[lvl].Hm, ls[lvl].Wm,
                                    desc->out_dims[lvl], desc->in_dims[lvl], desc->merge_h, desc->merge_w, ls[lvl].Hin, ls[lvl].Win,
@@ -1888,6 +1930,17 @@
     if (e != hipSuccess) return fail(SWF_ERR_HIP, "model_forward_checked: memset: %s", hipGetErrorString(e));
     return model_forward_impl(desc, arena, static_cast<const char*>(packed), ir, vis, out, B, H, W, workspace, workspace_bytes, stream,
                               cross_equal_flags);
+}
+
+int32_t swf_model_unmerge_tail_mask(const swf_model_desc* desc, int32_t B, int32_t H, int32_t W) {
+    if (check_model_desc(desc) != SWF_OK || B <= 0) return 0;
+    LevelShape ls[SWF_MAX_LEVELS];
+    if (model_shapes(desc, H, W, ls) != SWF_OK) return 0;
+    const PackedPlan plan = packed_plan(desc);
+    int32_t mask = 0;
+    for (int j = 0; j < desc->levels; ++j)
+        if (unmerge_tail_fused(desc, plan, ls, j, B)) mask |= 1 << (desc->levels - 1 - j);
+    return mask;
 }
 
 int swf_model_forward_profiled(const swf_model_desc* desc, const float* arena, const void* packed, const float* ir, const float* vis,
diff --git a/swin_unet_image_fusion_amd/csrc/win_host.h b/swin_unet_image_fusion_amd/csrc/win_host.h
--- a/swin_unet_image_fusion_amd/csrc/win_host.h
+++ b/swin_unet_image_fusion_amd/csrc/win_host.h
@@ -116,9 +116,35 @@
 }
 
 template <class L>
+int win_tail_cout(const swf_block_desc& d, int H, int W) {
+    (void)H; (void)W;
+    const bool ok = L::TAIL_COUT > 0 && win_supported<L>(d) && d.attn.win_h != 16 && d.hidden == L::HID_NARROW;
+    return ok ? L::TAIL_COUT : 0;
+}
+
+template <class L>
+int win_launch_tail(const swf_block_desc& d, WinArgs a, const WinTail& tail, int B, int H, int W, int nwin, hipStream_t stream) {
+    if (!win_tail_cout<L>(d, H, W)) return fail(SWF_ERR_UNSUPPORTED, "%s: no un-merge tail for this block", L::name);
+    uintptr_t bits = 0;
+    for (int s = 0; s < 2; ++s) {
+        if (!tail.out[s] || !tail.packed[s]) return fail(SWF_ERR_NULL, "%s: un-merge tail without output or packed image", L::name);
+        bits |= reinterpret_cast<uintptr_t>(tail.out[s]) | reinterpret_cast<uintptr_t>(tail.skip[s]) | reinterpret_cast<uintptr_t>(tail.packed[s]);
+    }
+    if (bits % 16) return fail(SWF_ERR_UNSUPPORTED, "%s: un-merge tail tensors must be 16-byte aligned", L::name);
+    if (tail.Hm <= 0 || tail.Wm <= 0 || tail.Hm > H || tail.Wm > W || tail.Ho <= 0 || tail.Wo <= 0 || tail.Ho > 2 * tail.Hm || tail.Wo > 2 * tail.Wm)
+        return fail(SWF_ERR_BAD_SHAPE, "%s: un-merge tail crop %dx%d of %dx%d, output %dx%d", L::name, tail.Hm, tail.Wm, H, W, tail.Ho, tail.Wo);
+    if ((int64_t)B * tail.Ho * tail.Wo * L::TAIL_COUT * 4 >= (int64_t(1) << 31))
+        return fail(SWF_ERR_UNSUPPORTED, "%s: un-merged map exceeds the 2 GB buffer window", L::name);
+    a.tail = tail;
+    const int grid = std::min(nwin, L::WAVES * num_cus());
+    if (d.attn.win_h != 8) return L::template launch<L::HID_NARROW, 7, WIN_BLOCK, false, WIN_TAIL_UNMERGE>(d, a, grid, stream);
+    return L::template launch<L::HID_NARROW, 8, WIN_BLOCK, false, WIN_TAIL_UNMERGE>(d, a, grid, stream);
+}
+
+template <class L>
 int win_launch(const swf_block_desc& d, const void* packed_x, const void* packed_y, const float* x_in, const float* y_in,
                float* x_out, float* y_out, int B, int H, int W, hipStream_t stream, const void* next_packed_x,
-               const void* next_packed_y, size_t next_bytes) {
+               const void* next_packed_y, size_t next_bytes, const WinTail* tail) {
     const int wsd = d.attn.win_h;
     if (!win_supported<L>(d) || H % wsd || W % wsd) return fail(SWF_ERR_UNSUPPORTED, "%s: shape not covered", L::name);
     if (!win_rows_fit<L>((int64_t)B * H * W))
@@ -128,13 +154,17 @@
     if (!a.warm[1]) a.warm[0] = nullptr;
     a.warm_bytes = (int)(next_bytes ? next_bytes : win_packed_bytes<L>(d));
     const int nwin = B * (H / wsd) * (W / wsd);
+    if (tail) {
+        if constexpr (L::TAIL_COUT > 0) return win_launch_tail<L>(d, a, *tail, B, H, W, nwin, stream);
+        else return fail(SWF_ERR_UNSUPPORTED, "%s: no un-merge tail at this level", L::name);
+    }
     if (wsd != 16) return win_launch_as<L, WIN_BLOCK, false>(d, a, nwin, stream);
     return d.hidden == L::HID_WIDE ? L::template launch16<L::HID_WIDE>(a, nwin, stream) : L::template launch16<L::HID_NARROW>(a, nwin, stream);
 }
 
 template <class L>
 constexpr WinLevel win_level() {
-    return {win_supported<L>, win_packed_bytes<L>, win_half_packed_bytes<L>, win_pack<L>, win_launch_half<L>, win_launch<L>};
+    return {win_supported<L>, win_packed_bytes<L>, win_half_packed_bytes<L>, win_pack<L>, win_launch_half<L>, win_launch<L>, win_tail_cout<L>};
 }
 
 }
diff --git a/swin_unet_image_fusion_amd/csrc/win_level.h b/swin_unet_image_fusion_amd/csrc/win_level.h
--- a/swin_unet_image_fusion_amd/csrc/win_level.h
+++ b/swin_unet_image_fusion_amd/csrc/win_level.h
@@ -2,6 +2,14 @@
 #include "swf_common.h"
 
 namespace swf {
+
+struct WinTail {
+    float* out[2];
+    const float* skip[2];
+    const char* packed[2];
+    int Hm, Wm;
+    int Ho, Wo;
+};
 
 struct WinArgs {
     const float* in[2];
@@ -10,9 +18,11 @@
     const char* warm[2];
     int B, H, W, shift, cross, warm_bytes;
     int ntok[2];
+    WinTail tail;
 };
 
 constexpr int WIN_BLOCK = 0, WIN_ATTN = 1, WIN_MLP = 2;
+constexpr int WIN_TAIL_NONE = 0, WIN_TAIL_UNMERGE = 1;
 
 struct WinPackArgs {
     swf_block_stream_params p[2];
@@ -30,7 +40,8 @@
                        const float* y_in, float* x_out, float* y_out, int B, int H, int W, int ntok_x, int ntok_y, hipStream_t stream);
     int (*launch)(const swf_block_desc& d, const void* packed_x, const void* packed_y, const float* x_in, const float* y_in,
                   float* x_out, float* y_out, int B, int H, int W, hipStream_t stream, const void* next_packed_x,
-                  const void* next_packed_y, size_t next_bytes);
+                  const void* next_packed_y, size_t next_bytes, const WinTail* tail);
+    int (*tail_cout)(const swf_block_desc& d, int H, int W);
 };
 
 const WinLevel& win24_level();
diff --git a/swin_unet_image_fusion_amd/csrc/win_tail.h b/swin_unet_image_fusion_amd/csrc/win_tail.h
--- /dev/null
+++ b/swin_unet_image_fusion_amd/csrc/win_tail.h
@@ -0,0 +1,138 @@
+#pragma once
+#include "win_frag.h"
+#include "win_level.h"
+
+namespace swf {
+namespace wf {
+
+template <int CIN, int COUT>
+struct WinTailG {
+    static constexpr int N = 4 * COUT, NKS = (CIN + 15) / 16, NT = (N + 31) / 32, NV = NT * 16;
+    static constexpr int NFRAG = NT * NKS * 2;
+    static constexpr size_t p_vec = size_t(NFRAG) * 1024, p_total = p_vec + size_t(3) * 2 * NV * 4;
+    static constexpr int LDS_FLOATS = 2 * 3 * 2 * NV;
+    static_assert(COUT == 1 || COUT % 4 == 0, "a lane's four channels lie in one output pixel");
+    static_assert(LDS_FLOATS % 8 == 0 && p_vec % 16 == 0, "vector sections move as 16-byte groups");
+    static_assert(NFRAG <= 18 && NT <= 3, "all fragments and all skip values of a token are in flight at once: registers");
+};
+
+template <class TG>
+__device__ __forceinline__ void tail_fill_vectors(float* tvec, const WinTail& t, int tid) {
+    fill_vectors<TG::LDS_FLOATS / 8, 256>(tvec, t.packed[0] + TG::p_vec, t.packed[1] + TG::p_vec, tid);
+}
+
+template <class TG>
+__device__ __forceinline__ void tail_request(const WinTail& t, int ws, int lane, u32x4 (&w)[TG::NFRAG]) {
+    asm volatile("" : "+s"(ws));
+    const __amdgpu_buffer_rsrc_t trs = __builtin_amdgcn_make_buffer_rsrc(const_cast<char*>(t.packed[ws]), 0, (int)TG::p_total, 0x00020000);
+    const unsigned loff = (unsigned)lane * 16u;
+    SWF_WF_FENCE();
+#pragma unroll
+    for (int i = 0; i < TG::NFRAG; ++i) w[i] = __builtin_bit_cast(u32x4, __builtin_amdgcn_raw_buffer_load_b128(trs, loff, i * 1024, 0));
+    SWF_WF_FENCE();
+}
+
+template <class TG, int COUT>
+__device__ __forceinline__ void unmerge_tail(const WinTail& t, int ws, const float* tvs, const u32x4 (&w)[TG::NFRAG], const float* n, int b, int my,
+                                             int mx, bool live, int lane, int out_bytes) {
+    constexpr int NT = TG::NT, NKS = TG::NKS, NV = TG::NV, N = TG::N;
+    constexpr unsigned NONE = 0x80000000u;
+    const int hf = lane >> 5;
+    asm volatile("" : "+s"(ws));
+    const float* skp = t.skip[ws];
+    const __amdgpu_buffer_rsrc_t srs = __builtin_amdgcn_make_buffer_rsrc(const_cast<float*>(skp), 0, skp ? out_bytes : 0, 0x00020000);
+    const __amdgpu_buffer_rsrc_t urs = __builtin_amdgcn_make_buffer_rsrc(t.out[ws], 0, out_bytes, 0x00020000);
+
+    unsigned pix[4];
+#pragma unroll
+    for (int pq = 0; pq < 4; ++pq) {
+        const int yy = 2 * my + (pq >> 1), xx = 2 * mx + (pq & 1);
+        pix[pq] = (live && yy < t.Ho && xx < t.Wo) ? (unsigned)((((b * t.Ho + yy) * t.Wo + xx) * COUT) * 4) : NONE;
+    }
+    constexpr bool VEC = COUT > 1;
+    unsigned voff[VEC ? NT : 1][4];
+    f32x4 skv[VEC ? NT : 1][4];
+    if constexpr (VEC) {
+#pragma unroll
+        for (int nt = 0; nt < NT; ++nt)
+#pragma unroll
+            for (int g = 0; g < 4; ++g) {
+                const int na = 32 * nt + 8 * g, nb = na + 4;
+                const unsigned oa = na < N ? pix[(na / COUT) & 3] + 4u * (unsigned)(na % COUT) : NONE;
+                const unsigned ob = nb < N ? pix[(nb / COUT) & 3] + 4u * (unsigned)(nb % COUT) : NONE;
+                voff[nt][g] = hf ? ob : oa;
+                skv[nt][g] = __builtin_bit_cast(f32x4, __builtin_amdgcn_raw_buffer_load_b128(srs, voff[nt][g], 0, 0));
+            }
+    }
+
+    u32x4 bh[NKS], bl[NKS];
+#pragma unroll
+    for (int ks = 0; ks < NKS; ++ks) split8(n + 8 * ks, bh[ks], bl[ks]);
+    const f32x16 zero16 = {0.f, 0.f, 0.f, 0.f, 0.f, 0.f, 0.f, 0.f, 0.f, 0.f, 0.f, 0.f, 0.f, 0.f, 0.f, 0.f};
+    f32x16 acc[NT];
+#pragma unroll
+    for (int nt = 0; nt < NT; ++nt) {
+        acc[nt] = zero16;
+#pragma unroll
+        for (int ks = 0; ks < NKS; ++ks) acc[nt] = mma3(w[(nt * NKS + ks) * 2], w[(nt * NKS + ks) * 2 + 1], bh[ks], bl[ks], acc[nt]);
+    }
+
+    const float* vbias = tvs + hf * NV;
+    const float* vgam = tvs + 2 * NV + hf * NV;
+    const float* vbet = tvs + 4 * NV + hf * NV;
+    constexpr float invN = 1.0f / (float)N;
+    float sum = 0.f;
+#pragma unroll
+    for (int nt = 0; nt < NT; ++nt)
+#pragma unroll
+        for (int i = 0; i < 16; ++i) {
+            acc[nt][i] += vbias[nt * 16 + i];
+            sum += acc[nt][i];
+        }
+    const float mean = sum_halves(sum) * invN;
+    float q = 0.f;
+#pragma unroll
+    for (int nt = 0; nt < NT; ++nt)
+#pragma unroll
+        for (int i = 0; i < 16; ++i) {
+            const float d = acc[nt][i] - mean;
+            q += (N % 32 == 0 || 32 * nt + rho(i, hf) < N) ? d * d : 0.f;
+        }
+    const float rstd = __builtin_amdgcn_rsqf(sum_halves(q) * invN + 1e-5f);
+#pragma unroll
+    for (int nt = 0; nt < NT; ++nt)
+#pragma unroll
+        for (int g = 0; g < 4; ++g) {
+            if (32 * nt + 8 * g < N) {
+                float y[4];
+#pragma unroll
+                for (int j = 0; j < 4; ++j) {
+                    const int i = 4 * g + j;
+                    const float z = (acc[nt][i] - mean) * rstd * vgam[nt * 16 + i] + vbet[nt * 16 + i];
+                    y[j] = z > 0.f ? z : __builtin_amdgcn_exp2f(z * kLog2e) - 1.0f;
+                }
+                if constexpr (VEC) {
+                    const f32x4 k4 = skv[nt][g];
+                    const f32x4 v = {y[0] + k4.x, y[1] + k4.y, y[2] + k4.z, y[3] + k4.w};
+                    __builtin_amdgcn_raw_buffer_store_b128(__builtin_bit_cast(u32x4, v), urs, voff[nt][g], 0, 0);
+                } else {
+                    float k1[4] = {0.f, 0.f, 0.f, 0.f};
+                    if (skp) {
+#pragma unroll
+                        for (int j = 0; j < 4; ++j) {
+                            const unsigned o = hf ? NONE : pix[j];
+                            k1[j] = __builtin_bit_cast(float, __builtin_amdgcn_raw_buffer_load_b32(srs, o, 0, 0));
+                        }
+                    }
+#pragma unroll
+                    for (int j = 0; j < 4; ++j) {
+                        const unsigned o = hf ? NONE : pix[j];
+                        __builtin_amdgcn_raw_buffer_store_b32(__builtin_bit_cast(unsigned, y[j] + k1[j]), urs, o, 0, 0);
+                    }
+                }
+            }
+        }
+}
+
+}
+}
```

Measured after the change: 9060 pairs/s (median of 6 runs). No clear change (+1.0%).
